# TheProParadox/3dspa_code

Measured on AMD Instinct MI355X. Metric: train-step tracks/sec (B x N_tracks) at T=150, C=772, higher is better.
Workload: dtype bf16

## Files before the change

### 3dspa_code_amd/_lib.py

```python
from __future__ import annotations

import ctypes as C
import os

HERE = os.path.dirname(os.path.abspath(__file__))
LIB_PATH = os.path.join(HERE, 'libspa3d_hip.so')

F32, BF16, F16 = 0, 1, 2


class Config(C.Structure):
  _fields_ = [
      ('num_output_frames', C.c_int32), ('num_latent_tokens', C.c_int32), ('latent_token_dim', C.c_int32),
      ('num_frequencies', C.c_int32), ('track_scale_factor', C.c_float), ('time_scale_factor', C.c_float),
      ('track_token_dim', C.c_int32), ('encoder_latent_dim', C.c_int32), ('decoder_num_channels', C.c_int32),
      ('dino_feature_dim', C.c_int32), ('depth_feature_dim', C.c_int32), ('num_heads', C.c_int32),
      ('qkv_size', C.c_int32), ('enc_mlp', C.c_int32), ('enc_layers', C.c_int32), ('t2l_mlp', C.c_int32),
      ('t2l_layers', C.c_int32), ('dec_mlp', C.c_int32), ('dec_layers', C.c_int32), ('ro_mlp', C.c_int32),
      ('ro_layers', C.c_int32), ('precision', C.c_int32), ('model_kind', C.c_int32),
  ]


class Batch(C.Structure):
  _fields_ = [
# ... 17 lines not shown

class LossConfig(C.Structure):
  _fields_ = [('l1_weight', C.c_float), ('bce_weight', C.c_float), ('position_kind', C.c_int32), ('huber_delta', C.c_float),
              ('axis_weight', C.c_float * 3), ('bce_pos_weight', C.c_float)]


class TapVid3D(C.Structure):
  _fields_ = [('scaling', C.c_int32), ('fixed_thresholds', C.c_int32), ('intrinsics', C.c_void_p), ('query_stats', C.c_void_p),
              ('sample_stats', C.c_void_p), ('scale', C.c_void_p), ('row_scale', C.c_void_p), ('ratio', C.c_void_p)]


class Render(C.Structure):
  _fields_ = [('N', C.c_int32), ('T', C.c_int32), ('H', C.c_int32), ('W', C.c_int32), ('video', C.c_void_p), ('out', C.c_void_p), ('tracks', C.c_void_p),
              ('coords', C.c_int32), ('intrinsics', C.c_void_p), ('extrinsics', C.c_void_p), ('resize_h', C.c_int32), ('resize_w', C.c_int32),
              ('scores', C.c_void_p), ('visible', C.c_void_p), ('normalize', C.c_int32), ('use_visibility', C.c_int32), ('colour_bgr', C.c_int32),
              ('trail', C.c_int32), ('point_size', C.c_int32), ('pixels', C.c_void_p)]


class Clip(C.Structure):
  _fields_ = [('n_tracks', C.c_int32), ('T', C.c_int32), ('H', C.c_int32), ('W', C.c_int32), ('tracks_2d', C.c_void_p), ('tracks_3d', C.c_void_p),
              ('visible', C.c_void_p), ('depth_map', C.c_void_p), ('dino_map', C.c_void_p), ('Hp', C.c_int32), ('Wp', C.c_int32), ('dino_pool', C.c_void_p),
              ('depth_pool', C.c_void_p), ('intrinsics', C.POINTER(C.c_double)), ('n_support', C.c_int32), ('n_query', C.c_int32),
              ('support_index', C.c_void_p), ('query_index', C.c_void_p), ('query_frame', C.c_void_p)]


_SIGS = {
    'spa3d_version': (C.c_char_p, []),
    'spa3d_create': (C.c_int, [C.POINTER(Config), C.POINTER(C.c_void_p)]),
    'spa3d_destroy': (C.c_int, [C.c_void_p]),
    'spa3d_last_error': (C.c_char_p, [C.c_void_p]),
    'spa3d_param_elems': (C.c_int64, [C.c_void_p]),
    'spa3d_num_leaves': (C.c_int32, [C.c_void_p]),
    'spa3d_leaf_info': (C.c_int, [C.c_void_p, C.c_int32, C.c_char_p, C.POINTER(C.c_int32), C.POINTER(C.c_int64),
                                  C.POINTER(C.c_int64)]),
    'spa3d_workspace_bytes': (C.c_int64, [C.c_void_p, C.c_int32, C.c_int32, C.c_int32, C.c_int32, C.c_int32, C.c_int32]),
    'spa3d_encode': (C.c_int, [C.c_void_p, C.c_void_p, C.POINTER(Batch), C.c_void_p, C.c_void_p, C.c_int64, C.c_void_p]),
    'spa3d_decode': (C.c_int, [C.c_void_p, C.c_void_p, C.POINTER(Batch), C.c_void_p, C.POINTER(Outputs), C.c_void_p,
                               C.c_int64, C.c_void_p]),
    'spa3d_forward': (C.c_int, [C.c_void_p, C.c_void_p, C.POINTER(Batch), C.POINTER(Outputs), C.c_void_p, C.c_int64,
                                C.c_void_p]),
    'spa3d_loss': (C.c_int, [C.c_void_p, C.POINTER(Batch), C.POINTER(Outputs), C.c_float, C.c_void_p, C.c_void_p]),
    'spa3d_score': (C.c_int, [C.c_void_p, C.c_void_p, C.POINTER(Batch), C.POINTER(Scores), C.POINTER(Outputs), C.c_void_p, C.c_int64,
                              C.c_void_p]),
    'spa3d_score_folds_workspace_bytes': (C.c_int64, [C.c_void_p, C.c_int32, C.c_int32, C.c_int32]),
    'spa3d_score_folds': (C.c_int, [C.c_void_p, C.c_void_p, C.POINTER(Batch), C.c_int32, C.POINTER(C.c_int32), C.POINTER(Scores), C.POINTER(Outputs),
                                    C.c_void_p, C.c_int64, C.c_void_p]),
    'spa3d_score_from_preds': (C.c_int, [C.c_void_p, C.POINTER(Batch), C.POINTER(Outputs), C.POINTER(Scores), C.c_void_p]),
    'spa3d_tapvid3d_workspace_bytes': (C.c_int64, [C.c_void_p, C.c_int32, C.c_int32, C.c_int32]),
    'spa3d_tapvid3d_from_preds': (C.c_int, [C.c_void_p, C.POINTER(Batch), C.POINTER(Outputs), C.POINTER(TapVid3D), C.c_void_p, C.c_int64, C.c_void_p]),
    'spa3d_render_workspace_bytes': (C.c_int64, [C.c_void_p, C.c_int32, C.c_int32]),
    'spa3d_render_tracks': (C.c_int, [C.c_void_p, C.POINTER(Render), C.c_void_p, C.c_int64, C.c_void_p]),
    'spa3d_build_batch': (C.c_int, [C.c_void_p, C.POINTER(Clip), C.POINTER(Batch), C.c_void_p]),
    'spa3d_op_median_rows': (C.c_int, [C.c_void_p, C.c_int64, C.c_int64, C.c_void_p, C.c_void_p, C.c_int64, C.c_void_p]),
    'spa3d_loss_and_grads': (C.c_int, [C.c_void_p, C.c_void_p, C.POINTER(Batch), C.c_float, C.c_void_p, C.c_int32,
                                       C.c_void_p, C.POINTER(Outputs), C.c_void_p, C.c_int64, C.c_void_p]),
    'spa3d_adamw_step': (C.c_int, [C.c_void_p, C.c_void_p, C.c_void_p, C.c_void_p, C.c_int64, C.c_float, C.c_int64,
                                   C.c_float, C.c_float, C.c_float, C.c_float, C.c_float, C.c_void_p, C.c_void_p]),
    'spa3d_set_option': (C.c_int, [C.c_void_p, C.c_char_p, C.c_double]),
    'spa3d_set_loss_scale_state': (C.c_int, [C.c_void_p, C.c_void_p]),
    'spa3d_set_counts': (C.c_int, [C.c_void_p, C.c_int32, C.POINTER(C.c_int32), C.POINTER(C.c_int32)]),
    'spa3d_set_loss': (C.c_int, [C.c_void_p, C.POINTER(LossConfig)]),
    'spa3d_get_loss': (C.c_int, [C.c_void_p, C.POINTER(LossConfig)]),
    'spa3d_set_point_weights': (C.c_int, [C.c_void_p, C.c_int32, C.c_int32, C.c_void_p]),
    'spa3d_grad_segments': (C.c_int, [C.c_void_p, C.POINTER(C.c_int64)]),
    'spa3d_trainable_range': (C.c_int, [C.c_void_p, C.POINTER(C.c_int64)]),
    'spa3d_set_grad_events': (C.c_int, [C.c_void_p, C.c_void_p, C.c_void_p]),
    'spa3d_grad_events_recorded': (C.c_int, [C.c_void_p, C.POINTER(C.c_int64)]),
    'spa3d_detach': (C.c_int, [C.c_void_p, C.c_void_p, C.c_void_p, C.c_void_p]),
    'spa3d_plan_stats': (C.c_int, [C.c_void_p, C.POINTER(C.c_double)]),
    'spa3d_prof_enable': (C.c_int, [C.c_void_p, C.c_int32]),
    'spa3d_prof_read': (C.c_int, [C.c_void_p, C.c_int32, C.POINTER(C.c_double)]),
    'spa3d_prof_dump': (C.c_int, [C.c_void_p, C.c_char_p]),
    'spa3d_uniform_noise': (C.c_int, [C.c_void_p, C.c_int64, C.c_uint32, C.c_uint32, C.c_void_p]),
    'spa3d_op_sin_embed': (C.c_int, [C.c_void_p, C.c_int64, C.c_int32, C.c_int32, C.c_void_p, C.c_int32, C.c_void_p]),
    'spa3d_op_linear': (C.c_int, [C.c_void_p, C.c_void_p, C.c_void_p, C.c_void_p, C.c_void_p, C.c_int64, C.c_int32,
                                  C.c_int32, C.c_int32, C.c_int32, C.c_int32, C.c_void_p, C.c_int64, C.c_void_p]),
    'spa3d_op_linear_bwd': (C.c_int, [C.c_void_p, C.c_void_p, C.c_void_p, C.c_void_p, C.c_void_p, C.c_void_p, C.c_int64,
                                      C.c_int32, C.c_int32, C.c_int32, C.c_int32, C.c_void_p, C.c_int64, C.c_void_p]),
    'spa3d_op_mlp_fused': (C.c_int, [C.c_void_p] * 9 + [C.c_int64, C.c_int32, C.c_int32, C.c_int32, C.c_void_p, C.c_int64, C.c_void_p]),
    'spa3d_op_layernorm': (C.c_int, [C.c_void_p, C.c_void_p, C.c_void_p, C.c_void_p, C.c_int64, C.c_int32, C.c_int32,
                                     C.c_void_p]),
    'spa3d_op_layernorm_bwd': (C.c_int, [C.c_void_p, C.c_void_p, C.c_void_p, C.c_void_p, C.c_void_p, C.c_void_p,
                                         C.c_int64, C.c_int32, C.c_int32, C.c_void_p]),
    'spa3d_op_qkv_attention': (C.c_int, [C.c_void_p, C.c_int64] + [C.c_void_p] * 7 + [C.c_int64, C.c_int32, C.c_int32] + [C.c_void_p] * 3
                               + [C.c_int32, C.c_void_p, C.c_int64, C.c_void_p]),
    'spa3d_op_attention': (C.c_int, [C.c_void_p] * 3 + [C.c_int64] * 3 + [C.c_void_p] * 3 + [C.c_int64] + [C.c_int32] * 4
                           + [C.c_void_p, C.c_void_p, C.c_int32, C.c_int32, C.c_void_p, C.c_int64, C.c_void_p]),
    'spa3d_op_attention_holdout': (C.c_int, [C.c_void_p] * 3 + [C.c_int64] * 3 + [C.c_void_p] * 2 + [C.c_int64] + [C.c_int32] * 4
                                   + [C.POINTER(C.c_int32), C.c_void_p, C.c_void_p, C.c_int32, C.c_int32, C.c_void_p, C.c_int64, C.c_void_p]),
    'spa3d_op_attention_bwd': (C.c_int, [C.c_void_p] * 3 + [C.c_int64] * 3 + [C.c_void_p] * 3 + [C.c_int64]
                               + [C.c_int32] * 4 + [C.c_void_p] * 8 + [C.c_int32, C.c_int32, C.c_void_p, C.c_int64,
                                                                       C.c_void_p]),
    'spa3d_op_attention_ragged': (C.c_int, [C.c_void_p] * 3 + [C.c_int64] * 3 + [C.c_void_p] * 3 + [C.POINTER(C.c_int32), C.c_int64] + [C.c_int32] * 3
                                  + [C.c_void_p, C.c_void_p, C.c_int32, C.c_int32, C.c_void_p, C.c_int64, C.c_void_p]),
    'spa3d_op_attention_ragged_bwd': (C.c_int, [C.c_void_p] * 3 + [C.c_int64] * 3 + [C.c_void_p] * 3 + [C.POINTER(C.c_int32), C.c_int64] + [C.c_int32] * 3
                                      + [C.c_void_p] * 8 + [C.c_int32, C.c_int32, C.c_void_p, C.c_int64, C.c_void_p]),
    'spa3d_op_attention_varlen': (C.c_int, [C.c_void_p] * 3 + [C.c_int64] * 3 + [C.c_void_p] * 2 + [C.POINTER(C.c_int32), C.c_int64] + [C.c_int32] * 3
                                  + [C.c_void_p, C.c_void_p, C.c_int32, C.c_int32, C.c_void_p, C.c_int64, C.c_void_p]),
    'spa3d_op_attention_varlen_bwd': (C.c_int, [C.c_void_p] * 3 + [C.c_int64] * 3 + [C.c_void_p] * 2 + [C.POINTER(C.c_int32), C.c_int64] + [C.c_int32] * 3
                                      + [C.c_void_p] * 8 + [C.c_int32, C.c_int32, C.c_void_p, C.c_int64, C.c_void_p]),
    'spa3d_op_attention_q1': (C.c_int, [C.c_void_p, C.c_int64, C.c_void_p, C.c_void_p, C.c_int64, C.c_int64] + [C.c_void_p] * 4 + [C.c_int64]
                              + [C.c_int32] * 3 + [C.c_void_p, C.c_void_p, C.c_int32, C.c_void_p]),
    'spa3d_op_attention_q1_bwd': (C.c_int, [C.c_void_p, C.c_int64, C.c_void_p, C.c_void_p, C.c_int64, C.c_int64] + [C.c_void_p] * 4 + [C.c_int64]
                                  + [C.c_int32] * 3 + [C.c_void_p] * 7 + [C.c_int32, C.c_void_p]),
    'spa3d_op_rank_linear': (C.c_int, [C.c_void_p] * 4 + [C.c_int64, C.c_int32, C.c_int32, C.c_int64, C.c_int32, C.c_int32, C.c_int32, C.c_void_p]),
    'spa3d_op_rank_linear_bwd': (C.c_int, [C.c_void_p, C.c_void_p, C.c_int64, C.c_int32, C.c_int32, C.c_int64, C.c_int32, C.c_int32, C.c_void_p,
                                           C.c_void_p, C.c_int32, C.c_void_p]),
    'spa3d_op_colsum': (C.c_int, [C.c_void_p, C.c_int64, C.c_int32, C.c_int64, C.c_int32, C.c_int32, C.c_void_p, C.c_int32, C.c_void_p]),
    'spa3d_op_rows': (C.c_int, [C.c_int32, C.c_void_p, C.c_void_p, C.c_int64, C.c_void_p, C.c_int64, C.c_int32, C.c_int32, C.c_void_p]),
    'spa3d_op_prune_plan': (C.c_int, [C.c_void_p, C.c_int64, C.c_int32, C.c_void_p, C.c_void_p, C.c_void_p, C.POINTER(C.c_int64), C.c_void_p]),
    'spa3d_op_share_plan': (C.c_int, [C.c_void_p, C.c_int64, C.c_int32] + [C.c_void_p] * 5 + [C.POINTER(C.c_int64), C.c_void_p]),
    'spa3d_op_share_rows': (C.c_int, [C.c_int32] + [C.c_void_p] * 6 + [C.c_int64, C.c_int64] + [C.c_int32] * 4 + [C.c_void_p, C.c_int32, C.c_void_p]),
    'spa3d_op_assemble_readout': (C.c_int, [C.c_void_p] * 3 + [C.c_int64] + [C.c_int32] * 4 + [C.c_void_p, C.c_int32, C.c_void_p]),
    'spa3d_op_assemble_readout_bwd': (C.c_int, [C.c_void_p] * 2 + [C.c_int64] + [C.c_int32] * 4 + [C.c_void_p, C.c_void_p, C.c_int32, C.c_int32, C.c_void_p]),
    'spa3d_op_broadcast_rows': (C.c_int, [C.c_void_p, C.c_int32, C.c_int32, C.c_void_p, C.c_int64, C.c_int32, C.c_void_p]),
    'spa3d_op_bcast_grad': (C.c_int, [C.c_void_p, C.c_int64, C.c_int64, C.c_int64, C.c_void_p, C.c_int32, C.c_void_p]),
    'spa3d_op_vis_mean_pool': (C.c_int, [C.c_void_p, C.c_void_p, C.c_int64, C.c_int32, C.c_int32, C.c_void_p, C.c_int32, C.c_void_p]),
    'spa3d_op_vis_mean_pool_bwd': (C.c_int, [C.c_void_p, C.c_void_p, C.c_int64, C.c_int32, C.c_int32, C.c_void_p, C.c_int32, C.c_void_p]),
    'spa3d_op_sin_embed_scaled': (C.c_int, [C.c_void_p, C.c_int64, C.c_int32, C.c_int32, C.c_float, C.c_void_p, C.c_int32, C.c_void_p]),
    'spa3d_op_embed_tokens': (C.c_int, [C.c_void_p, C.c_int64, C.c_int32, C.c_int32, C.c_int32, C.c_float, C.c_void_p, C.c_int32, C.c_void_p]),
    'spa3d_op_query_embed': (C.c_int, [C.c_void_p, C.c_int64, C.c_int32, C.c_int32, C.c_float, C.c_float, C.c_void_p, C.c_void_p, C.c_void_p]),
    'spa3d_op_embed_maps': (C.c_int, [C.c_void_p, C.c_int64, C.c_int32, C.c_int32] + [C.c_void_p] * 4 + [C.c_int32, C.c_int32, C.c_void_p]),
    'spa3d_op_set_readout_rows': (C.c_int, [C.c_void_p, C.c_void_p, C.c_int64, C.c_int32, C.c_int32, C.c_int32, C.c_void_p]),
    'spa3d_op_keymask': (C.c_int, [C.c_void_p, C.c_void_p, C.c_int64, C.c_int32, C.c_int32, C.c_int32, C.c_void_p, C.c_void_p]),
    'spa3d_op_sum3': (C.c_int, [C.c_void_p] * 4 + [C.c_int32, C.c_void_p]),
    'spa3d_op_pack': (C.c_int, [C.c_void_p, C.c_int64, C.c_int32, C.c_int32, C.c_void_p, C.c_int64, C.c_void_p, C.c_int64, C.c_int32, C.c_void_p]),
    'spa3d_op_transpose': (C.c_int, [C.c_void_p, C.c_int32, C.c_int32, C.c_void_p, C.c_int32, C.c_void_p]),
    'spa3d_op_discretize': (C.c_int, [C.c_void_p, C.c_void_p, C.c_int32, C.c_void_p, C.c_void_p, C.c_int64, C.c_void_p]),
    'spa3d_op_sample_dino': (C.c_int, [C.c_void_p, C.c_void_p] + [C.c_int32] * 7 + [C.c_void_p, C.c_int32, C.c_void_p]),
    'spa3d_op_sample_depth_features': (C.c_int, [C.c_void_p, C.c_void_p] + [C.c_int32] * 4 + [C.c_void_p, C.c_void_p]),
    'spa3d_op_lift_2d_to_3d': (C.c_int, [C.c_void_p, C.c_void_p] + [C.c_int32] * 4 + [C.POINTER(C.c_double), C.c_void_p, C.c_void_p]),
}

_lib = None


def exported_symbols():
  return sorted(_SIGS)


def load():
  global _lib
  if _lib is not None:
    return _lib
  if not os.path.exists(LIB_PATH):
    raise ImportError(
        f'{LIB_PATH} is missing: build it with `python -c "import __graft_entry__ as g; g.build()"` '
        '(hipcc --offload-arch=gfx950).  The 3DSPA hot path has no CPU fallback.')
  lib = C.CDLL(LIB_PATH)
  for name, (res, args) in _SIGS.items():
    fn = getattr(lib, name)
    fn.restype = res
    fn.argtypes = args
  _lib = lib
  return lib


class Spa3dError(RuntimeError):
  pass


def check(rc, handle=None, what=''):
  if rc != 0:
    msg = ''
    if handle is not None:
      msg = load().spa3d_last_error(handle).decode()
# ... 2 lines not shown
```

### 3dspa_code_amd/csrc/common.hpp

```cpp
#pragma once
#include <hip/hip_runtime.h>
#include <stdint.h>
#include <algorithm>
#include <string>
#include <vector>

#include "../../include/spa3d.h"
#include "ablate.inc"
#include "gemm_plan.hpp"
#include "attn_plan.hpp"
#include "score_row.hpp"
#include "loss_point.hpp"

#ifndef SPA_F16
#define SPA_F16 0
#endif
#if SPA_F16
#define SPA_NS h_f16
#else
#define SPA_NS h_bf16
#endif
typedef unsigned short bf16_t;

struct DetCfg { float* gbase; long long* shadow; long long n; unsigned* flag; float scale; };
// ... 118 lines not shown

struct ScoreArgs {
  const float* head; const float* tracks; const float* vlog;
  const float* tgt; const float* tvis; const float* scale;
  float* qstats; float* frame_err;
  int64_t nq, row0; int Q, T, NC; ScoreThr thr;
};

constexpr int RENDER_CHUNK = 256;

struct Leaf {
  std::string name;
  int ndim;
  int64_t shape[4];
  int64_t offset;
  int64_t numel() const { int64_t n = 1; for (int i = 0; i < ndim; ++i) n *= shape[i]; return n; }
};

struct Arena {
  char* base = nullptr;
  int64_t cap = 0, off = 0, peak = 0;
  bool dry = false, overflow = false;
  void* alloc(int64_t bytes) {
    int64_t a = (off + 255) & ~int64_t(255);
    off = a + bytes;
    if (off > peak) peak = off;
    if (dry) return (void*)(uintptr_t)(0x1000 + a);
    if (off > cap) { overflow = true; return base; }
    return base + a;
  }
  int64_t mark() const { return off; }
  void release(int64_t m) { off = m; }
};

enum { PROF_GEMM_NT = 0, PROF_GEMM_TN = 1, PROF_GEMM_GENERIC = 2, PROF_ATTN_FWD = 3, PROF_ATTN_BWD = 4, PROF_LN_FWD = 5, PROF_LN_BWD = 6,
       PROF_ATTN_Q1 = 7, PROF_EMBED = 8, PROF_NCLS = 9 };
struct ProfRec { int cls; double flops, bytes; hipEvent_t e0, e1; int64_t tag[4] = {0, 0, 0, 0}; };
struct Prof {
  bool on = false;
  std::vector<hipEvent_t> pool; size_t used = 0;
  std::vector<ProfRec> recs;
  hipEvent_t get() {
    if (used == pool.size()) { hipEvent_t e; if (hipEventCreate(&e) != hipSuccess) return nullptr; pool.push_back(e); }
    return pool[used++];
  }
};

inline spa3d_loss_config loss_config_defaults() {
  spa3d_loss_config d;
  d.l1_weight = 5000.0f; d.bce_weight = 1e-8f; d.position_kind = SPA3D_POS_L1; d.huber_delta = 1.f;
  d.axis_weight[0] = d.axis_weight[1] = d.axis_weight[2] = 1.f; d.bce_pos_weight = 1.f;
  return d;
}

struct spa3d_ctx {
  spa3d_config cfg;
  std::vector<Leaf> leaves;
  int64_t nparams = 0;
  std::string err;
  hipStream_t stream = nullptr;
  Arena ar;
  bool dry = false;
  int hip_err = 0;
  GemmPolicy gemm;
  AttnPolicy attn;
  int chunk = 0;
  int query_chunk = 0;
  int track_chunk = 0;
  int ro_share = 1;
  int prune = 1;
  float loss_scale = 1.f;
  void* grad_ev[2] = {nullptr, nullptr};
  int64_t grad_ev_gen[2] = {0, 0};
  bool last_chunk = false;
  const float* loss_scale_state = nullptr;
  double plan_stats[4] = {0, 0, 0, 0};
  int det_grads = 0;
  const DetCfg* det = nullptr;
  std::vector<int32_t> cnt_n, cnt_q; bool has_cnt_n = false, has_cnt_q = false; int cnt_B = 0;
  spa3d_loss_config loss = loss_config_defaults(); float loss_gmax = 5000.f; int loss_gshift = 0;
  const float* pt_w = nullptr; int pt_B = 0, pt_Q = 0;
  int poison = 0;
  int freeze = 0;
  Prof prof;
};

template <typename F> inline int64_t arena_peak(spa3d_ctx* c, F&& body) {
  const Arena saved = c->ar; const bool sd = c->dry;
  c->ar = Arena(); c->ar.dry = true; c->dry = true;
  body();
  const int64_t peak = c->ar.peak;
  c->ar = saved; c->dry = sd;
  return peak;
}
template <typename F> inline int sized_call(spa3d_ctx* c, const char* what, int64_t need, void* ws, int64_t ws_bytes, void* stream, F&& body) {
  if (!ws || ws_bytes < need) { c->err = std::string(what) + ": workspace too small: need " + std::to_string(need) + " bytes"; return SPA3D_ERR_ARG; }
  c->stream = (hipStream_t)stream; c->dry = false;
  c->ar = Arena(); c->ar.base = (char*)ws; c->ar.cap = ws_bytes;
  body();
  if (c->ar.overflow) { c->err = "internal: arena overflow"; return SPA3D_ERR_WORKSPACE; }
  return c->hip_err ? SPA3D_ERR_HIP : SPA3D_OK;
}
inline bool counts_fit_batch(spa3d_ctx* c, int B) {
  if (c->cnt_B == B) return true;
  c->err = "counts were set for B = " + std::to_string(c->cnt_B) + ", this batch has B = " + std::to_string(B);
  return false;
}
inline bool weights_fit_batch(spa3d_ctx* c, int B, int Q) {
  if (!c->pt_w || (c->pt_B == B && c->pt_Q == Q)) return true;
  c->err = "point weights were set for B = " + std::to_string(c->pt_B) + ", Q = " + std::to_string(c->pt_Q) + ", this batch has B = " + std::to_string(B) +
           ", Q = " + std::to_string(Q);
  return false;
}
inline const int32_t* checked_query_counts(spa3d_ctx* c, int B, int Q) {
  if (!counts_fit_batch(c, B)) return nullptr;
  for (int i = 0; i < B; ++i)
    if (c->cnt_q[i] < 0 || c->cnt_q[i] > Q) {
      c->err = "query_count[" + std::to_string(i) + "] = " + std::to_string(c->cnt_q[i]) + " is outside [0, Q = " + std::to_string(Q) + "]";
      return nullptr;
    }
  return c->cnt_q.data();
}
template <typename F> inline void for_each_live_span(const int32_t* cq, int64_t B, int64_t Q, F&& f) {
  if (!cq) { f((int64_t)0, B * Q); return; }
  for (int64_t i = 0; i < B; ++i) f(i * Q, (int64_t)cq[i]);
}

struct ProfScope {
  spa3d_ctx* c; ProfRec r; bool on;
  ProfScope(spa3d_ctx* c_, int cls, double flops, double bytes) : c(c_), on(c_->prof.on && !c_->dry) {
    if (!on) return;
    r.cls = cls; r.flops = flops; r.bytes = bytes; r.e0 = c->prof.get(); r.e1 = c->prof.get();
    if (!r.e0 || !r.e1) { on = false; return; }
    (void)hipEventRecord(r.e0, c->stream);
  }
  void tag(int64_t a, int64_t b, int64_t c2, int64_t d) { r.tag[0] = a; r.tag[1] = b; r.tag[2] = c2; r.tag[3] = d; }
  ~ProfScope() { if (on) { (void)hipEventRecord(r.e1, c->stream); c->prof.recs.push_back(r); } }
};

#define SPA_LAUNCH_CHECK(ctx)                                                     \
  do {                                                                            \
    hipError_t e__ = hipGetLastError();                                           \
    if (e__ != hipSuccess && (ctx)->hip_err == 0) {                               \
      (ctx)->hip_err = (int)e__;                                                  \
      (ctx)->err = std::string("HIP launch failed at ") + __FILE__ + ":" +        \
                   std::to_string(__LINE__) + ": " + hipGetErrorString(e__);      \
    }                                                                             \
  } while (0)

#define GRID1D(n, bs) dim3((unsigned)std::min<int64_t>(((n) + (bs)-1) / (bs), 1 << 20))
static inline int64_t cdiv(int64_t a, int64_t b) { return (a + b - 1) / b; }

namespace SPA_NS {
template <typename T> void gemm_generic(spa3d_ctx* c, const GemmDesc& d);
void gemm_nt_bf16(spa3d_ctx* c, const GemmDesc& d, GemmKernel k);
void gemm_tn_bf16(spa3d_ctx* c, const GemmDesc& d, GemmKernel k);
int64_t gemm_ntb_pack_elems(int K, int N);
template <typename S> void gemm_ntb_pack(spa3d_ctx* c, const S* w, int64_t sk, int64_t sn, int K, int N, bf16_t* wpk);
void gemm_ntb(spa3d_ctx* c, const GemmDesc& d);
int64_t gemm_rs_pack_elems(int N);
template <typename S> void gemm_rs_pack(spa3d_ctx* c, const S* w, int64_t sk, int64_t sn, int N, bf16_t* wpk);
void gemm_rs(spa3d_ctx* c, const GemmDesc& d);
int64_t qkv_attn_pack_elems(int H);
template <typename S> void qkv_attn_pack(spa3d_ctx* c, const S* wq, const S* wk, const S* wv , int E, int H, bf16_t* wpk);
void qkv_attn_launch(spa3d_ctx* c, const AttnDesc& d);
void attn_fused_launch(spa3d_ctx* c, const AttnDesc& d, const AttnPlan& pl, float* const part[2]);
template <typename S> void mlp_fused_pack(spa3d_ctx* c, const S* w_in , const S* w_out , bf16_t* wpk);
int64_t mlp_fused_pack_elems();
void mlp_fused_fwd(spa3d_ctx* c, const bf16_t* na, const bf16_t* a, bf16_t* y, bf16_t* h, bf16_t* hpre, int64_t M, const bf16_t* wpk,
                   const float* b_in, const float* b_out);
template <typename T> void gemm_launch(spa3d_ctx* c, const GemmDesc& d, GemmKernel k) {
  if (c->dry) return;
  if constexpr (sizeof(T) == 2) {
    if (k == GemmKernel::Rs) return gemm_rs(c, d);
    if (k == GemmKernel::Ntb) return gemm_ntb(c, d);
    if (gemm_is_tn(k)) return gemm_tn_bf16(c, d, k);
    if (k != GemmKernel::Generic) return gemm_nt_bf16(c, d, k);
  }
  gemm_generic<T>(c, d);
}

template <typename T> void k_layernorm(spa3d_ctx*, const T* x, const float* scale, T* y, float* stats, int64_t rows, int d);
template <typename T> void k_layernorm_bwd(spa3d_ctx*, const T* x, const float* scale, const float* stats, const T* dy, T* dx,
                                           float* dscale, int64_t rows, int d, const T* add);
template <typename T> void attention_fwd(spa3d_ctx* c, const AttnDesc& d);
template <typename T> void attention_bwd(spa3d_ctx* c, const AttnDesc& d);
void attn_launch(spa3d_ctx* c, const AttnDesc& d, const AttnPlan& pl);
template <typename T> void k_sin_embed(spa3d_ctx*, const float* x, int64_t rows, int C, int nf, float prescale, T* out);
template <typename T> void k_embed_tokens(spa3d_ctx*, const float* tracks, int64_t nrows, int T_, int nf, float prescale, T* sinbuf, int NC = 3);
void k_query_embed1(spa3d_ctx*, const float* qp, int64_t nq, int nf, float track_scale, float time_scale, float* feat, int32_t* qframe,
                    int NC = 3);
template <typename T> void k_embed_maps(spa3d_ctx*, const int32_t* row_src, int64_t rows, int S, int T_, int32_t* arow, int32_t* crow, T* tok, const float* readout, int d);
template <typename T> void k_set_readout_rows(spa3d_ctx*, T* tok, const float* readout, int64_t nseq, int S, int d);
void k_keymask(spa3d_ctx*, const float* visible, const int32_t* boundary, int64_t nseq, int N, int T_, float* km);
void k_keymask2d(spa3d_ctx*, const float* visible, const int32_t* boundary, int64_t nseq, int N, int T_, float* km);
void k_sum3(spa3d_ctx*, const float* a, const float* b, const float* c3, float* out, int n);
template <typename T> bool k_rank_fwd(spa3d_ctx*, const T* x, const T* w , const float* bias, T* out , int64_t M, int N, int K, int64_t ldo,
                                      int rgroup, int rskip);
template <typename T> bool k_rank_bwd(spa3d_ctx*, const T* x, const T* dy, int64_t M, int N, int K, int64_t ldy, int rgroup, int rskip, float* gw ,
                                      float* gb );
template <typename T> void k_pack(spa3d_ctx*, const float* src, int64_t src_ld, int rows, int cols, T* dst_native, int64_t ldn, T* dst_T, int64_t ldt);
template <typename T> void k_transpose(spa3d_ctx*, const T* src, int rows, int cols, T* dst);
void k_zero(spa3d_ctx*, void* p, int64_t bytes);
void k_set_i32(spa3d_ctx*, int32_t* dst, const int32_t* host, int64_t n);
void k_mul(spa3d_ctx*, float* a, const float* b, int64_t n);
template <typename T> void k_cast_from_f32(spa3d_ctx*, const float* src, T* dst, int64_t n);
template <typename T> void k_cast_to_f32(spa3d_ctx*, const T* src, float* dst, int64_t n);
template <typename T> void k_colsum(spa3d_ctx*, const T* x, int64_t rows, int n, int64_t ld, float* out , int rgroup = 0,
                                    int rskip = 0);
template <typename T> void k_gather_rows(spa3d_ctx*, const T* src, int64_t src_stride_rows, T* dst, int64_t n, int d);
template <typename T> void k_rows_idx(spa3d_ctx*, int mode , const T* src, const int32_t* idx, T* dst, int64_t n, int d);
template <typename T> void k_add_rows_strided(spa3d_ctx*, T* dst, const T* src, int64_t dst_stride_rows, int64_t n, int d);
int64_t k_prune_plan(spa3d_ctx*, const float* km, int64_t nseq, int S, int32_t* cnt, int32_t* seq_off, int32_t* row_src);
int64_t k_share_plan(spa3d_ctx*, const int32_t* qframe, int64_t B, int Q, int32_t* slot, int32_t* slot_b, int32_t* slot_f, int32_t* slot_q0, int32_t* scratch);
template <typename T> void k_share_assemble(spa3d_ctx*, const T* qtok, const T* lat, const int32_t* slot_b, const int32_t* slot_f, int64_t nslot, int64_t BQ,
                                            int L, int Cl, int D, T* xU);
template <typename T> void k_share_expand(spa3d_ctx*, const T* srcU, const int32_t* slot, const int32_t* slot_q0, int64_t nslot, int64_t nseq, int S, int d,
                                          const T* add, T* dst);
template <typename T> void k_share_reduce(spa3d_ctx*, const T* src, const int32_t* slot, const int32_t* slot_b, int64_t nslot, int64_t nseq, int Q, int S, int d,
                                          T* dstU);
template <typename T> void k_assemble_readout(spa3d_ctx*, const T* qtok, const T* lat, const int32_t* qframe, int64_t B, int Q, int L, int Cl,
                                              int D, T* seq);
template <typename T> void k_assemble_readout_bwd(spa3d_ctx*, const T* dseq, const int32_t* qframe, int64_t B, int Q, int L, int Cl, int D,
                                                  T* dqtok, float* dlat, bool accumulate = false);
template <typename T> void k_broadcast_rows(spa3d_ctx*, const float* src, int rows, int d, T* dst, int64_t B);
template <typename T> void k_bcast_grad(spa3d_ctx*, const T* dsrc, int64_t per, int64_t B, int64_t bstride, float* dparam);
template <typename T> void k_vis_mean_pool(spa3d_ctx*, const T* tok, const float* vis, int64_t nseq, int T_, int d, T* out);
template <typename T> void k_vis_mean_pool_bwd(spa3d_ctx*, const T* dout, const float* vis, int64_t nseq, int T_, int d, T* dtok);
template <typename T> void k_attn_q1_fwd(spa3d_ctx*, const T* q0, int64_t ldq0, const T* k, const T* v, int64_t ldk, int64_t ldv,
                                         const float* sq, const float* sk, const float* km, int64_t nseq, int S, int H, int Dh, T* o0,
                                         float* p0, const int32_t* seq_off = nullptr);
template <typename T> void k_attn_q1_bwd(spa3d_ctx*, const T* q0, int64_t ldq0, const T* k, const T* v, int64_t ldk, int64_t ldv,
                                         const float* sq, const float* sk, const float* km, int64_t nseq, int S, int H, int Dh,
                                         const float* p0, const T* d_o0, T* dq0, T* dk, T* dv, float* dsq, float* dsk,
                                         const int32_t* seq_off = nullptr);
void k_discretize(spa3d_ctx*, const float* lat, const float* noise, int discretize, float* out, float* clipmask, int64_t n);
void k_loss_fwd(spa3d_ctx*, const float* head, int64_t nq, int T_, const float* tgt, const float* tvis, float* tracks, float* vlog,
                float* clog, float* sums, unsigned* poison, int NC, const spa3d_loss_config& lc, const float* wgt);
void k_loss_from_preds(spa3d_ctx*, const float* tracks, const float* vlog, int64_t n, const float* tgt, const float* tvis, float* sums,
                       unsigned* poison, int NC, const spa3d_loss_config& lc, const float* wgt);
void k_score_rows(spa3d_ctx*, const ScoreArgs& a);
void k_score_reduce(spa3d_ctx*, const float* qstats, int64_t B, int Q, int K, double* out );
void k_vis_count(spa3d_ctx*, const float* tvis, int64_t n, float* out, unsigned* poison);
void k_set_denom(spa3d_ctx*, const float* sums, const unsigned* poison, float denom_host, float* denom_dev);
void k_loss_finalize(spa3d_ctx*, const float* sums, const unsigned* poison, const float* denom_dev, float l1w, float bcew, float* loss3);
template <typename T> void k_loss_bwd(spa3d_ctx*, const float* head, int64_t nq, int T_, const float* tgt, const float* tvis,
                                      const float* denom_dev, const spa3d_loss_config& lc, const float* wgt, T* dhead, int NC = 3,
                                      const float* scale_dev = nullptr);
void k_set_loss_scale(spa3d_ctx*, const float* denom_dev, float gmax, float setting, float* scale_dev);
void k_unscale(spa3d_ctx*, float* a, const float* scale_dev, int64_t n);
void k_adamw(spa3d_ctx*, float* p, const float* g, float* m, float* v, int64_t n, float lr, int64_t step, float clip, float b1, float b2,
             float eps, float wd, float* scratch);
void k_uniform_noise(spa3d_ctx*, float* out, int64_t n, uint32_t k0, uint32_t k1);
void k_det_flush(spa3d_ctx* c, int64_t lo, int64_t n);
void k_det_unit(spa3d_ctx*, const float* sums, const unsigned* poison, const float* denom_dev, const float* scale_dev, int gshift, const DetCfg& d, DetCfg* out);
}
using namespace SPA_NS;
```

### 3dspa_code_amd/csrc/layernorm.hip

```cpp
#include <algorithm>

#include "common.hpp"

namespace SPA_NS {

template <typename T>
__global__ __launch_bounds__(256) void ln_fwd_kernel(const T* __restrict__ x, const float* __restrict__ scale, T* __restrict__ y,
                                                     float* __restrict__ stats, int64_t rows, int d) {
  const int lane = threadIdx.x & 63;
  int64_t row = (int64_t)blockIdx.x * 4 + (threadIdx.x >> 6);
  const int64_t stride = (int64_t)gridDim.x * 4;
  for (; row < rows; row += stride) {
    const T* xr = x + row * d;
    float s = 0.f, ss = 0.f;
    for (int i = lane; i < d; i += 64) { float v = ld(xr + i); s += v; ss += v * v; }
    s = wave_sum(s); ss = wave_sum(ss);
    float mu = s / d;
    float var = fmaxf(ss / d - mu * mu, 0.f);
    float r = rsqrtf(var + 1e-6f);
    if (stats && lane == 0) { stats[row * 2] = mu; stats[row * 2 + 1] = r; }
    T* yr = y + row * d;
    for (int i = lane; i < d; i += 64) st(yr + i, (ld(xr + i) - mu) * r * scale[i]);
  }
}
#define LN_MAXJ 32
template <typename T>
__global__ __launch_bounds__(256) void ln_bwd_kernel(const T* __restrict__ x, const float* __restrict__ scale,
                                                     const float* __restrict__ stats, const T* __restrict__ dy, const T* add,
                                                     T* dx, float* __restrict__ dscale, int64_t rows, int d, const DetCfg* det) {
  __shared__ float red[4][64 * LN_MAXJ / 4];
  const int lane = threadIdx.x & 63, w = threadIdx.x >> 6;
  float acc[LN_MAXJ];
#pragma unroll
  for (int j = 0; j < LN_MAXJ; ++j) acc[j] = 0.f;
  int64_t row = (int64_t)blockIdx.x * 4 + w;
  const int64_t stride = (int64_t)gridDim.x * 4;
  for (; row < rows; row += stride) {
    const T* xr = x + row * d;
    const T* dyr = dy + row * d;
    const float mu = stats[row * 2], r = stats[row * 2 + 1];
    float sg = 0.f, sgx = 0.f;
#pragma unroll
    for (int j = 0; j < LN_MAXJ; ++j) {
      int i = lane + 64 * j;
      if (i < d) {
        float xh = (ld(xr + i) - mu) * r;
        float dyv = ld(dyr + i);
        float g = dyv * scale[i];
        sg += g; sgx += g * xh;
        acc[j] += dyv * xh;
      }
    }
    sg = wave_sum(sg) / d; sgx = wave_sum(sgx) / d;
    T* dxr = dx + row * d;
#pragma unroll
    for (int j = 0; j < LN_MAXJ; ++j) {
      int i = lane + 64 * j;
      if (i < d) {
        float xh = (ld(xr + i) - mu) * r;
        float g = ld(dyr + i) * scale[i];
        float v = r * (g - sg - xh * sgx);
        if (add) v += ld(add + row * d + i);
        st(dxr + i, v);
      }
    }
  }
  for (int j0 = 0; j0 < LN_MAXJ; j0 += 8) {
    if (j0 * 64 >= d) break;
    __syncthreads();
#pragma unroll
    for (int j = 0; j < 8; ++j) red[w][j * 64 + lane] = acc[j0 + j];
    __syncthreads();
    if (w == 0) {
#pragma unroll
      for (int j = 0; j < 8; ++j) {
        int i = lane + 64 * (j0 + j);
        if (i < d) {
          float s = red[0][j * 64 + lane] + red[1][j * 64 + lane] + red[2][j * 64 + lane] + red[3][j * 64 + lane];
          grad_add(det_read(det), dscale + i, s);
        }
      }
    }
  }
}
template <typename T, int NV>
__device__ __forceinline__ void unpack_vec(const uint4& v, float (&f)[NV]) {
  if constexpr (sizeof(T) == 4) { f[0] = __uint_as_float(v.x); f[1] = __uint_as_float(v.y); f[2] = __uint_as_float(v.z); f[3] = __uint_as_float(v.w); }
  else { const unsigned u[4] = {v.x, v.y, v.z, v.w};
#pragma unroll
    for (int i = 0; i < 4; ++i) { f[2 * i] = unpack_lo(u[i]); f[2 * i + 1] = unpack_hi(u[i]); } }
}
template <typename T, int STEPS, int U = 2>
__global__ __launch_bounds__(256) void ln_fwd_vec_kernel(const T* __restrict__ x, const float* __restrict__ scale, T* __restrict__ y,
                                                         float* __restrict__ stats, int64_t rows, int d) {
  constexpr int NV = VecOf<T>::N;
  const int lane = threadIdx.x & 63, w = threadIdx.x >> 6;
  const int nch = d / NV;
  float sc[STEPS][NV];
#pragma unroll
  for (int s_ = 0; s_ < STEPS; ++s_) {
    const int c = lane + 64 * s_;
#pragma unroll
    for (int j = 0; j < NV; ++j) sc[s_][j] = c < nch ? scale[c * NV + j] : 0.f;
  }
  const int64_t stride = (int64_t)gridDim.x * 4;
  for (int64_t row0 = (int64_t)blockIdx.x * 4 + w; row0 < rows; row0 += stride * U) {
    float xv[U][STEPS][NV];
#pragma unroll
    for (int u = 0; u < U; ++u) {
      const int64_t row = row0 + u * stride;
#pragma unroll
      for (int s_ = 0; s_ < STEPS; ++s_) {
        const int c = lane + 64 * s_;
        if (row < rows && c < nch) load_vec<T, NV>(x + row * d + c * NV, xv[u][s_]);
        else {
#pragma unroll
          for (int j = 0; j < NV; ++j) xv[u][s_][j] = 0.f;
        }
      }
    }
#pragma unroll
    for (int u = 0; u < U; ++u) {
      const int64_t row = row0 + u * stride;
      float s = 0.f, ss = 0.f;
#pragma unroll
      for (int s_ = 0; s_ < STEPS; ++s_)
#pragma unroll
        for (int j = 0; j < NV; ++j) { s += xv[u][s_][j]; ss += xv[u][s_][j] * xv[u][s_][j]; }
      s = wave_sum(s); ss = wave_sum(ss);
      const float mu = s / d;
      const float var = fmaxf(ss / d - mu * mu, 0.f);
      const float r = rsqrtf(var + 1e-6f);
      if (row < rows) {
        if (stats && lane == 0) { stats[row * 2] = mu; stats[row * 2 + 1] = r; }
#pragma unroll
        for (int s_ = 0; s_ < STEPS; ++s_) {
          const int c = lane + 64 * s_;
          if (c < nch) {
            float o[NV];
#pragma unroll
            for (int j = 0; j < NV; ++j) o[j] = (xv[u][s_][j] - mu) * r * sc[s_][j];
            store_vec<T, NV>(y + row * d + c * NV, o);
          }
        }
      }
    }
  }
}
template <typename T, int LPR, int CH>
__global__ __launch_bounds__(256) void ln_fwd_part_kernel(const T* __restrict__ x, const float* __restrict__ scale, T* __restrict__ y,
                                                          float* __restrict__ stats, int64_t rows, int d) {
  constexpr int NV = VecOf<T>::N, RPB = 256 / LPR;
  const int sub = threadIdx.x & (LPR - 1);
  float sc[CH][NV];
#pragma unroll
  for (int c = 0; c < CH; ++c)
#pragma unroll
    for (int j = 0; j < NV; ++j) sc[c][j] = scale[(sub + LPR * c) * NV + j];
  for (int64_t row = (int64_t)blockIdx.x * RPB + threadIdx.x / LPR; row < rows; row += (int64_t)gridDim.x * RPB) {
    uint4 xr[CH];
#pragma unroll
    for (int c = 0; c < CH; ++c) xr[c] = *(const uint4*)(x + row * d + (sub + LPR * c) * NV);
    float xv[CH][NV]; float s = 0.f, ss = 0.f;
#pragma unroll
    for (int c = 0; c < CH; ++c) {
      unpack_vec<T, NV>(xr[c], xv[c]);
#pragma unroll
      for (int j = 0; j < NV; ++j) { s += xv[c][j]; ss += xv[c][j] * xv[c][j]; }
    }
#pragma unroll
    for (int o = 1; o < LPR; o <<= 1) { s += __shfl_xor(s, o, 64); ss += __shfl_xor(ss, o, 64); }
    const float mu = s / d;
    const float var = fmaxf(ss / d - mu * mu, 0.f);
    const float r = rsqrtf(var + 1e-6f);
    if (stats && sub == 0) { stats[row * 2] = mu; stats[row * 2 + 1] = r; }
#pragma unroll
    for (int c = 0; c < CH; ++c) {
      float o[NV];
#pragma unroll
      for (int j = 0; j < NV; ++j) o[j] = (xv[c][j] - mu) * r * sc[c][j];
      store_vec<T, NV>(y + row * d + (sub + LPR * c) * NV, o);
    }
  }
}
template <typename T, int LPR, int CH>
__global__ __launch_bounds__(256) void ln_bwd_part_kernel(const T* __restrict__ x, const float* __restrict__ scale, const float* __restrict__ stats,
                                                          const T* __restrict__ dy, const T* add, T* dx, float* __restrict__ dscale, int64_t rows, int d,
                                                          const DetCfg* det) {
  constexpr int NV = VecOf<T>::N, RPB = 256 / LPR, DV = LPR * CH * NV;
  __shared__ float red[4][DV];
  const int lane = threadIdx.x & 63, w = threadIdx.x >> 6, sub = threadIdx.x & (LPR - 1);
  float acc[CH][NV], sc[CH][NV];
#pragma unroll
  for (int c = 0; c < CH; ++c)
#pragma unroll
    for (int j = 0; j < NV; ++j) { acc[c][j] = 0.f; sc[c][j] = scale[(sub + LPR * c) * NV + j]; }
  for (int64_t row = (int64_t)blockIdx.x * RPB + threadIdx.x / LPR; row < rows; row += (int64_t)gridDim.x * RPB) {
    uint4 xr[CH], dr[CH], ar[CH];
    const float mu = stats[row * 2], r = stats[row * 2 + 1];
#pragma unroll
    for (int c = 0; c < CH; ++c) {
      const int64_t o = row * d + (sub + LPR * c) * NV;
      xr[c] = *(const uint4*)(x + o); dr[c] = *(const uint4*)(dy + o);
      ar[c] = add ? *(const uint4*)(add + o) : make_uint4(0u, 0u, 0u, 0u);
    }
    float xh[CH][NV], gg[CH][NV]; float sg = 0.f, sgx = 0.f;
#pragma unroll
    for (int c = 0; c < CH; ++c) {
      float xv[NV], dv[NV];
      unpack_vec<T, NV>(xr[c], xv); unpack_vec<T, NV>(dr[c], dv);
#pragma unroll
      for (int j = 0; j < NV; ++j) {
        xh[c][j] = (xv[j] - mu) * r; gg[c][j] = dv[j] * sc[c][j];
        sg += gg[c][j]; sgx += gg[c][j] * xh[c][j]; acc[c][j] += dv[j] * xh[c][j];
      }
    }
#pragma unroll
    for (int o = 1; o < LPR; o <<= 1) { sg += __shfl_xor(sg, o, 64); sgx += __shfl_xor(sgx, o, 64); }
    sg /= d; sgx /= d;
#pragma unroll
    for (int c = 0; c < CH; ++c) {
      float o[NV], av[NV];
      unpack_vec<T, NV>(ar[c], av);
#pragma unroll
      for (int j = 0; j < NV; ++j) o[j] = r * (gg[c][j] - sg - xh[c][j] * sgx) + av[j];
      store_vec<T, NV>(dx + row * d + (sub + LPR * c) * NV, o);
    }
  }
#pragma unroll
  for (int c = 0; c < CH; ++c)
#pragma unroll
    for (int j = 0; j < NV; ++j) {
      float a = acc[c][j];
#pragma unroll
      for (int o = LPR; o < 64; o <<= 1) a += __shfl_xor(a, o, 64);
      if (lane < LPR) red[w][(sub + LPR * c) * NV + j] = a;
    }
  __syncthreads();
  for (int t = threadIdx.x; t < DV; t += 256) grad_add(det_read(det), dscale + t, red[0][t] + red[1][t] + red[2][t] + red[3][t]);
}
template <typename T>
void k_layernorm(spa3d_ctx* c, const T* x, const float* scale, T* y, float* stats, int64_t rows, int d) {
  if (c->dry || rows == 0) return;
  ProfScope ps(c, PROF_LN_FWD, 8.0 * (double)rows * d, (double)rows * d * 2.0 * sizeof(T) + rows * 8.0);
  ps.tag(rows, d, 0, 0);
  constexpr int NV = VecOf<T>::N;
  const bool al = ((((uintptr_t)x) | ((uintptr_t)y)) & 15) == 0;
  if (d % NV == 0 && al && d <= 64 * NV * 4) {
    constexpr int gcap = 4096;
    const unsigned g = (unsigned)std::min<int64_t>(cdiv(rows, 8), gcap);
    const int steps = (d / NV + 63) / 64;
    if constexpr (sizeof(T) == 2) {
      if (d == 384) { ln_fwd_part_kernel<T, 16, 3><<<(unsigned)std::min<int64_t>(cdiv(rows, 16), 2 * gcap), 256, 0, c->stream>>>(x, scale, y, stats, rows, d); SPA_LAUNCH_CHECK(c); return; }
      if (d == 1280) { ln_fwd_part_kernel<T, 32, 5><<<(unsigned)std::min<int64_t>(cdiv(rows, 8), 2 * gcap), 256, 0, c->stream>>>(x, scale, y, stats, rows, d); SPA_LAUNCH_CHECK(c); return; }
    }
    if (steps == 1) ln_fwd_vec_kernel<T, 1><<<g, 256, 0, c->stream>>>(x, scale, y, stats, rows, d);
    else if (steps == 2) ln_fwd_vec_kernel<T, 2><<<g, 256, 0, c->stream>>>(x, scale, y, stats, rows, d);
    else if (steps == 3) ln_fwd_vec_kernel<T, 3><<<g, 256, 0, c->stream>>>(x, scale, y, stats, rows, d);
    else ln_fwd_vec_kernel<T, 4><<<g, 256, 0, c->stream>>>(x, scale, y, stats, rows, d);
  } else {
    const unsigned g = (unsigned)std::min<int64_t>(cdiv(rows, 4), 65536);
    ln_fwd_kernel<T><<<g, 256, 0, c->stream>>>(x, scale, y, stats, rows, d);
  }
  SPA_LAUNCH_CHECK(c);
}

template <typename T, int STEPS, int U>
__global__ __launch_bounds__(256) void ln_bwd_vec_kernel(const T* __restrict__ x, const float* __restrict__ scale,
                                                         const float* __restrict__ stats, const T* __restrict__ dy, const T* add, T* dx,
                                                         float* __restrict__ dscale, int64_t rows, int d, const DetCfg* det) {
  constexpr int NV = VecOf<T>::N;
  __shared__ float red[4][64 * NV];
  const int lane = threadIdx.x & 63, w = threadIdx.x >> 6;
  const int nch = d / NV;
  float acc[STEPS][NV], sc[STEPS][NV];
#pragma unroll
  for (int s_ = 0; s_ < STEPS; ++s_) {
    const int c = lane + 64 * s_;
#pragma unroll
    for (int j = 0; j < NV; ++j) { acc[s_][j] = 0.f; sc[s_][j] = c < nch ? scale[c * NV + j] : 0.f; }
  }
  const int64_t stride = (int64_t)gridDim.x * 4;
  for (int64_t row0 = (int64_t)blockIdx.x * 4 + w; row0 < rows; row0 += stride * U) {
    uint4 xr[U][STEPS], dr[U][STEPS], ar[U][STEPS]; float mu[U], r[U];
#pragma unroll
    for (int u = 0; u < U; ++u) {
      const int64_t row = row0 + u * stride;
      const bool live = row < rows;
      mu[u] = live ? stats[row * 2] : 0.f; r[u] = live ? stats[row * 2 + 1] : 0.f;
#pragma unroll
      for (int s_ = 0; s_ < STEPS; ++s_) {
        const int c = lane + 64 * s_;
        xr[u][s_] = dr[u][s_] = ar[u][s_] = make_uint4(0u, 0u, 0u, 0u);
        if (live && c < nch) {
          xr[u][s_] = *(const uint4*)(x + row * d + c * NV); dr[u][s_] = *(const uint4*)(dy + row * d + c * NV);
          if (add) ar[u][s_] = *(const uint4*)(add + row * d + c * NV);
        }
      }
    }
#pragma unroll
    for (int u = 0; u < U; ++u) {
      const int64_t row = row0 + u * stride;
      float xh[STEPS][NV], gg[STEPS][NV];
      float sg = 0.f, sgx = 0.f;
#pragma unroll
      for (int s_ = 0; s_ < STEPS; ++s_) {
        float xv[NV], dv[NV];
        unpack_vec<T, NV>(xr[u][s_], xv); unpack_vec<T, NV>(dr[u][s_], dv);
#pragma unroll
        for (int j = 0; j < NV; ++j) {
          xh[s_][j] = (xv[j] - mu[u]) * r[u]; gg[s_][j] = dv[j] * sc[s_][j];
          sg += gg[s_][j]; sgx += gg[s_][j] * xh[s_][j]; acc[s_][j] += dv[j] * xh[s_][j];
        }
      }
      sg = wave_sum(sg) / d; sgx = wave_sum(sgx) / d;
      if (row < rows) {
#pragma unroll
        for (int s_ = 0; s_ < STEPS; ++s_) {
          const int c = lane + 64 * s_;
          if (c < nch) {
            float o[NV], av[NV];
            unpack_vec<T, NV>(ar[u][s_], av);
#pragma unroll
            for (int j = 0; j < NV; ++j) o[j] = r[u] * (gg[s_][j] - sg - xh[s_][j] * sgx) + av[j];
            store_vec<T, NV>(dx + row * d + c * NV, o);
          }
        }
      }
    }
  }
#pragma unroll
  for (int s_ = 0; s_ < STEPS; ++s_) {
    __syncthreads();
#pragma unroll
    for (int j = 0; j < NV; ++j) red[w][lane * NV + j] = acc[s_][j];
    __syncthreads();
    if (w == 0) {
      const int c = lane + 64 * s_;
      if (c < nch)
#pragma unroll
        for (int j = 0; j < NV; ++j)
          grad_add(det_read(det), dscale + c * NV + j, red[0][lane * NV + j] + red[1][lane * NV + j] + red[2][lane * NV + j] + red[3][lane * NV + j]);
    }
  }
}
template <typename T>
void k_layernorm_bwd(spa3d_ctx* c, const T* x, const float* scale, const float* stats, const T* dy, T* dx, float* dscale,
                     int64_t rows, int d, const T* add) {
  if (c->dry || rows == 0) return;
  ProfScope ps(c, PROF_LN_BWD, 16.0 * (double)rows * d, (double)rows * d * (add ? 4.0 : 3.0) * sizeof(T) + rows * 8.0);
  ps.tag(rows, d, add ? 1 : 0, 0);
  constexpr int gcapb = 1024;
  unsigned g = (unsigned)std::min<int64_t>(cdiv(rows, 4), d <= 512 ? gcapb : 2 * gcapb);
  if (rows <= 16384) g = (unsigned)std::min<int64_t>(g, std::max<int64_t>(64, cdiv(rows, 32)));
  constexpr int NV = VecOf<T>::N;
  const bool al = ((((uintptr_t)x) | ((uintptr_t)dy) | ((uintptr_t)dx) | ((uintptr_t)add)) & 15) == 0;
  if (d % NV == 0 && al && d <= 64 * NV * 4) {
    const int steps = (d / NV + 63) / 64;
    if constexpr (sizeof(T) == 2) {
      if (d == 384) { ln_bwd_part_kernel<T, 16, 3><<<(unsigned)std::min<int64_t>(cdiv(rows, 16), 2 * gcapb), 256, 0, c->stream>>>(x, scale, stats, dy, add, dx, dscale, rows, d, c->det); SPA_LAUNCH_CHECK(c); return; }
      if (d == 1280) { ln_bwd_part_kernel<T, 32, 5><<<(unsigned)std::min<int64_t>(cdiv(rows, 8), 2 * gcapb), 256, 0, c->stream>>>(x, scale, stats, dy, add, dx, dscale, rows, d, c->det); SPA_LAUNCH_CHECK(c); return; }
    }
    if (steps == 1) ln_bwd_vec_kernel<T, 1, 1><<<g, 256, 0, c->stream>>>(x, scale, stats, dy, add, dx, dscale, rows, d, c->det);
    else if (steps == 2) ln_bwd_vec_kernel<T, 2, 2><<<g, 256, 0, c->stream>>>(x, scale, stats, dy, add, dx, dscale, rows, d, c->det);
    else if (steps == 3) ln_bwd_vec_kernel<T, 3, 2><<<g, 256, 0, c->stream>>>(x, scale, stats, dy, add, dx, dscale, rows, d, c->det);
    else ln_bwd_vec_kernel<T, 4, 1><<<g, 256, 0, c->stream>>>(x, scale, stats, dy, add, dx, dscale, rows, d, c->det);
  } else {
    ln_bwd_kernel<T><<<g, 256, 0, c->stream>>>(x, scale, stats, dy, add, dx, dscale, rows, d, c->det);
  }
  SPA_LAUNCH_CHECK(c);
}

#define INST_LN(T) \
  template void k_layernorm<T>(spa3d_ctx*, const T*, const float*, T*, float*, int64_t, int);                                        \
  template void k_layernorm_bwd<T>(spa3d_ctx*, const T*, const float*, const float*, const T*, T*, float*, int64_t, int, const T*);
INST_LN(float)
INST_LN(bf16_t)
}
```

### 3dspa_code_amd/csrc/model.hip

```cpp
#include <algorithm>
#include <cmath>
#include <cstring>
#include <map>

#include "common.hpp"
#include <cstdio>

enum { MODE_FORWARD = 0, MODE_TRAIN = 1, MODE_ENCODE = 2, MODE_DECODE = 3 };

struct RunArgs {
  int mode; const float* P; const spa3d_batch* b; float denom; float* G; int accumulate; float* loss3; spa3d_outputs* out;
  const float* latents_in; float* latents_out; int chunk;
  const int32_t* cn; const int32_t* cq;
  const spa3d_scores* score;
  const float* w;
  int nfold; const int32_t* fold_off;
};

namespace SPA_NS {
static inline const float* at_rows(const float* w, int64_t off) { return w ? w + off : nullptr; }

template <typename T> struct Lin {
  T* wn = nullptr;
  T* wt = nullptr;
// ... 92 lines not shown
      std::string b = name + "/layer_" + std::to_string(i);
      BlockW<T> w; w.d = d; w.mlp = mlp; w.cross = kv > 0; w.dkv = kv;
      w.norm_q = p(b + "/norm_q/scale"); w.g_norm_q = gr(b + "/norm_q/scale");
      w.norm_attn = p(b + "/norm_attn/scale"); w.g_norm_attn = gr(b + "/norm_attn/scale");
      std::string s = b + "/self_att";
      w.qkv = make_lin({s + "/dense_query/kernel", s + "/dense_key/kernel", s + "/dense_value/kernel"}, "", d, E);
      w.sq = p(s + "/norm_query/scale"); w.g_sq = gr(s + "/norm_query/scale");
      w.sk = p(s + "/norm_key/scale"); w.g_sk = gr(s + "/norm_key/scale");
      w.out = make_lin({s + "/dense_out/kernel"}, s + "/dense_out/bias", E, d);
      if (kv) {
        std::string x2 = b + "/cross_att";
        w.cq = make_lin({x2 + "/dense_query/kernel"}, "", d, E);
        w.ckv = make_lin({x2 + "/dense_key/kernel", x2 + "/dense_value/kernel"}, "", kv, E);
        w.csq = p(x2 + "/norm_query/scale"); w.g_csq = gr(x2 + "/norm_query/scale");
        w.csk = p(x2 + "/norm_key/scale"); w.g_csk = gr(x2 + "/norm_key/scale");
        w.cout = make_lin({x2 + "/dense_out/kernel"}, x2 + "/dense_out/bias", E, d);
      }
      w.mlp_in = make_lin({b + "/MLP_in/kernel"}, b + "/MLP_in/bias", d, mlp);
      w.mlp_out = make_lin({b + "/MLP_out/kernel"}, b + "/MLP_out/bias", mlp, d);
      if constexpr (sizeof(T) == 2) {
        if (plan_mlp_pack(c->gemm, w.cross, d, mlp)) {
          w.mlp_pk = alloc<T>(mlp_fused_pack_elems());
          mlp_fused_pack<float>(c, w.mlp_in.src[0], w.mlp_out.src[0], w.mlp_pk);
        }
        if (plan_qkv_pack(c->attn, c->gemm.generic, w.cross, d, Dh)) {
          w.qkv_pk = alloc<T>(qkv_attn_pack_elems(H));
          qkv_attn_pack<float>(c, w.qkv.src[0], w.qkv.src[1], w.qkv.src[2], E, H, w.qkv_pk);
        }
      }
      x.blocks.push_back(w);
    }
    x.norm_enc = p(name + "/norm_encoder/scale"); x.g_norm_enc = gr(name + "/norm_encoder/scale");
    return x;
  }
  void pack() {
    zero_page = c->ar.alloc(256); k_zero(c, zero_page, 256);
    const int d = g.track_token_dim, dl = g.encoder_latent_dim, dd = g.decoder_num_channels, nf = g.num_frequencies;
    lat0 = p("initializer/state_init"); g_lat0 = gr("initializer/state_init");
    readout = nullptr; g_readout = nullptr;
    if (!twoD) { readout = p("input_readout_token/state_init"); g_readout = gr("input_readout_token/state_init"); }
    tok = make_lin({"track_token_projection/kernel"}, "track_token_projection/bias", (NC + 1) * 2 * nf, d);
    if (g.dino_feature_dim > 0) dino = make_lin({"dino_projection/kernel"}, "dino_projection/bias", g.dino_feature_dim, d);
    if (g.depth_feature_dim > 0) depth = make_lin({"depth_projection/kernel"}, "depth_projection/bias", g.depth_feature_dim, d);
    if constexpr (sizeof(T) == 2) {
      if (plan_embed_pack(c->gemm, twoD, d, tok.K, g.dino_feature_dim, g.depth_feature_dim)) {
        emb_K = tok.K + (g.dino_feature_dim > 0 ? dino.K : 0);
        emb_wt = alloc<T>((int64_t)d * emb_K); emb_bias = alloc<float>(d);
        k_pack<T>(c, tok.src[0], d, tok.K, d, nullptr, 0, emb_wt, emb_K);
        if (g.dino_feature_dim > 0) k_pack<T>(c, dino.src[0], d, dino.K, d, nullptr, 0, emb_wt + tok.K, emb_K);
        k_sum3(c, tok.bias, g.dino_feature_dim > 0 ? dino.bias : nullptr, g.depth_feature_dim > 0 ? depth.bias : nullptr, emb_bias, d);
      }
    }
    enc = make_xf("input_track_transformer", d, g.enc_mlp, g.enc_layers, 0);
    t2l = make_xf("tracks_to_latents", dl, g.t2l_mlp, g.t2l_layers, d);
    comp = make_lin({"compressor/kernel"}, "compressor/bias", dl, g.latent_token_dim);
    decomp = make_lin({"decompressor/kernel"}, "decompressor/bias", g.latent_token_dim, dd - 128);
    dec = make_xf("decompress_attn", dd - 128, g.dec_mlp, g.dec_layers, 0);
    ro = make_xf("track_readout_attn", dd, g.ro_mlp, g.ro_layers, 0);
    qenc = make_lin({"query_encoder/kernel"}, "query_encoder/bias", (NC * 2 * nf + 1) * 2 * nf, dd);
    pred = make_lin({"track_predictor/kernel"}, "track_predictor/bias", dd, 4 * g.num_output_frames);
  }

  GemmKernel plan(const GemmDesc& d) const { return sizeof(T) == 2 ? plan_gemm(d, c->gemm) : GemmKernel::Generic; }
  void gemm(const GemmDesc& d) { gemm_launch<T>(c, d, plan(d)); }
  void lin_fwd(const Lin<T>& l, const T* X, void* Y, int64_t M, int epi = EPI_NONE, const T* residual = nullptr, int out_f32 = 0,
               int accumulate = 0, int64_t ldx = 0, int64_t ldy = 0, int crow_group = 0, int crow_skip = 0, T* pre_out = nullptr) {
    GemmDesc d{};
    d.A = X; d.B = l.wn; d.C = Y; d.M = M; d.N = l.N; d.K = l.K;
    d.sAm = ldx ? ldx : l.K; d.sAk = 1; d.sBk = l.ldn; d.sBn = 1; d.sCm = ldy ? ldy : l.N;
    d.Bt = l.wt; d.ldBt = l.K; d.rs_pk = l.wpk; d.ntb_pk = l.wnb;
    d.crow_group = crow_group; d.crow_skip = crow_skip; d.pre_out = pre_out;
    d.bias = l.bias; d.epi = epi; d.aux = residual; d.out_f32 = out_f32; d.accumulate = accumulate;
    gemm(d);
  }
  void lin_bwd_x(const Lin<T>& l, const T* dY, T* dX, int64_t M, const T* gelu_pre = nullptr, int accumulate = 0, int64_t lddx = 0) {
    GemmDesc d{};
    d.A = dY; d.B = l.wn; d.C = dX; d.M = M; d.N = l.K; d.K = l.N;
    d.sAm = l.N; d.sAk = 1; d.sBk = 1; d.sBn = l.ldn; d.sCm = lddx ? lddx : l.K;
    d.Bt = l.wn; d.ldBt = l.ldn; d.rs_pk = l.wpk_t; d.ntb_pk = l.wnb_t;
    if (gelu_pre) { d.epi = EPI_MUL_GELU_GRAD; d.aux = gelu_pre; }
    d.accumulate = accumulate;
    gemm(d);
  }
  void lin_bwd_w(const Lin<T>& l, const T* X, const T* dY, int64_t M, int64_t ldx = 0, int brow_group = 0, int brow_skip = 0) {
    if constexpr (sizeof(T) == 2) {
      if (l.nseg > 1 && !l.gb && l.gw[0]) {
        GemmDesc d{};
        d.A = X; d.B = dY; d.C = l.gw[0]; d.M = l.K; d.N = l.N; d.K = M;
        d.sAm = 1; d.sAk = ldx ? ldx : l.K; d.sBk = l.N; d.sBn = 1; d.sCm = l.segw;
        d.out_f32 = 1; d.accumulate = 1; d.zero_page = zero_page; d.brow_group = brow_group; d.brow_skip = brow_skip;
        d.seg_n = l.segw; d.C_seg[0] = l.gw[1]; d.C_seg[1] = l.nseg > 2 ? l.gw[2] : nullptr;
        const GemmKernel k = plan_tn(d, c->gemm);
        if (k != GemmKernel::Refuse) { gemm_launch<T>(c, d, k); return; }
      }
    }
    for (int s = 0; s < l.nseg; ++s) {
      GemmDesc d{};
      d.A = X; d.B = dY + (int64_t)s * l.segw; d.C = l.gw[s]; d.M = l.K; d.N = l.segw; d.K = M;
      d.sAm = 1; d.sAk = ldx ? ldx : l.K; d.sBk = l.N; d.sBn = 1; d.sCm = l.segw;
      d.out_f32 = 1; d.accumulate = 1; d.zero_page = zero_page; d.brow_group = brow_group; d.brow_skip = brow_skip;
      d.colsum_out = l.gb ? l.gb + (int64_t)s * l.segw : nullptr;
      const GemmKernel k = plan(d);
      gemm_launch<T>(c, d, k);
      if (l.gb && !gemm_tn_fuses_colsum(k, d)) k_colsum<T>(c, dY + (int64_t)s * l.segw, M, l.segw, l.N, l.gb + (int64_t)s * l.segw, brow_group, brow_skip);
    }
  }

  AttnDesc self_desc(const BlockW<T>& w, const T* qkv, T* o, float* lse, const float* km, int64_t nseq, int S, const Rag& rg, const T* d_o = nullptr,
                     T* dqkv = nullptr) {
    AttnDesc a;
    a.q = qkv; a.k = qkv + E; a.v = qkv + 2 * E; a.ldq = a.ldk = a.ldv = 3 * E; a.sq = w.sq; a.sk = w.sk; a.km = km; a.o = o; a.lse = lse;
    a.nseq = nseq; a.Sq = a.Sk = S; a.H = H; a.Dh = Dh; a.esz = (int)sizeof(T);
    if (rg.off) { a.layout = AttnLayout::RaggedRows; a.seq_off = rg.off; a.total_rows = rg.rows; }
    if (d_o) { a.d_o = d_o; a.dq = dqkv; a.dk = dqkv + E; a.dv = dqkv + 2 * E; a.dsq = w.g_sq; a.dsk = w.g_sk; }
    return a;
  }
  AttnDesc cross_desc(const BlockW<T>& w, const T* cq, const T* ckv, T* co, float* clse, int64_t nseq, int S, int Skv, const int32_t* koff_h,
                      const int32_t* koff_d, const Holes* hl, const T* d_o = nullptr, T* dcq = nullptr, T* dckv = nullptr) {
    AttnDesc a;
    a.q = cq; a.k = ckv; a.v = ckv + E; a.ldq = E; a.ldk = a.ldv = 2 * E; a.sq = w.csq; a.sk = w.csk; a.o = co; a.lse = clse;
    a.nseq = nseq; a.Sq = S; a.Sk = Skv; a.H = H; a.Dh = Dh; a.esz = (int)sizeof(T);
    if (hl) { a.layout = AttnLayout::Hole; a.holes_host = hl->host; a.holes_dev = hl->dev; a.Nk = hl->Nk; }
    else if (koff_h) { a.layout = AttnLayout::RaggedKeys; a.koff_host = koff_h; a.koff_dev = koff_d; }
    if (d_o) { a.d_o = d_o; a.dq = dcq; a.dk = dckv; a.dv = dckv + E; a.dsq = w.g_csq; a.dsk = w.g_csk; }
    return a;
  }

  void block_fwd(const BlockW<T>& w, const T* x, T* y, int64_t nseq, int S, const float* km, const T* kv, int Skv, BlockStash<T>* st,
                 const Rag& rg = Rag(), const Share<T>* sh = nullptr, const int32_t* koff_h = nullptr, const int32_t* koff_d = nullptr,
                 const Holes* hl = nullptr) {
    const int64_t M = rg.off ? rg.rows : nseq * S, Mg = rg.off ? (M + 7) & ~int64_t(7) : M; const int d = w.d;
    int64_t mk = c->ar.mark();
    T *nq, *qkv; float* st1;
    if (sh && sh->probe) sh = nullptr;
    if (sh) {
      const int64_t MU = sh->rows(nseq, S), MUg = (MU + 7) & ~int64_t(7);
      nq = alloc<T>(MUg * d); st1 = alloc<float>(MU * 2);
      k_layernorm<T>(c, sh->xU, w.norm_q, nq, st1, MU, d);
      qkv = alloc<T>(Mg * 3 * E);
      const int64_t mk2 = c->ar.mark();
      T* qkvU = alloc<T>(MUg * 3 * E);
      lin_fwd(w.qkv, nq, qkvU, MUg);
      k_share_expand<T>(c, qkvU, sh->slot, sh->slot_q0, sh->nslot, nseq, S, 3 * E, nullptr, qkv);
      c->ar.release(mk2);
    } else {
      nq = alloc<T>(Mg * d); st1 = alloc<float>(M * 2);
      k_layernorm<T>(c, x, w.norm_q, nq, st1, M, d);
      qkv = alloc<T>(Mg * 3 * E);
    }
    T* o = alloc<T>(Mg * E); float* lse = alloc<float>(M * H * 2);
    AttnDesc sa = self_desc(w, qkv, o, lse, km, nseq, S, rg);
    if (!sh) { sa.x = nq; sa.ldx = d; sa.d = d; sa.qkv_pk = w.qkv_pk; }
    const AttnPlan qa = plan_qkv_attn(sa, c->attn);
    if (qa.kernel == AttnKernel::QkvFwd) attn_launch(c, sa, qa);
    else {
      if (!sh) lin_fwd(w.qkv, nq, qkv, Mg);
      attention_fwd<T>(c, sa);
    }
    T* a = alloc<T>(Mg * d);
    lin_fwd(w.out, o, a, Mg, EPI_NONE, x);
    T *cq = nullptr, *ckv = nullptr, *co = nullptr; float* clse = nullptr;
    if (w.cross) {
      cq = alloc<T>(M * E); lin_fwd(w.cq, nq, cq, M);
      const int64_t nkv = hl ? hl->Nk : (koff_h ? koff_h[nseq] : nseq * Skv);
      ckv = alloc<T>(nkv * 2 * E); lin_fwd(w.ckv, kv, ckv, nkv);
      co = alloc<T>(M * E); clse = alloc<float>(M * H * 2);
      attention_fwd<T>(c, cross_desc(w, cq, ckv, co, clse, nseq, S, Skv, koff_h, koff_d, hl));
      lin_fwd(w.cout, co, a, M, EPI_NONE, a);
    }
    T* na = alloc<T>(Mg * d); float* st2 = alloc<float>(Mg * 2);
    k_layernorm<T>(c, a, w.norm_attn, na, st2, M, d);
    T* hpre = alloc<T>(Mg * w.mlp); T* h = alloc<T>(Mg * w.mlp);
    bool fused = false;
    if constexpr (sizeof(T) == 2) {
      fused = plan_mlp(c->gemm, Mg, d, w.mlp, w.mlp_pk, w.mlp_in.bias, w.mlp_out.bias, na, a, y, h, hpre) == GemmKernel::MlpFused;
      if (fused && !c->dry) mlp_fused_fwd(c, na, a, y, h, hpre, Mg, w.mlp_pk, w.mlp_in.bias, w.mlp_out.bias);
    }
    if (!fused) {
      lin_fwd(w.mlp_in, na, h, Mg, EPI_GELU, nullptr, 0, 0, 0, 0, 0, 0, hpre);
      lin_fwd(w.mlp_out, h, y, Mg, EPI_NONE, a);
    }
    if (st) { st->x = const_cast<T*>(sh ? sh->xU : x); st->nq = nq; st->qkv = qkv; st->o = o; st->a = a; st->na = na; st->hpre = hpre; st->h = h;
              st->st1 = st1; st->st2 = st2; st->cq = cq; st->ckv = ckv; st->co = co; st->lse = lse; st->clse = clse; st->shared = sh != nullptr; }
    else c->ar.release(mk);
  }
  void block_bwd(const BlockW<T>& w, const BlockStash<T>& s, const T* dy, T* dx, int64_t nseq, int S, const float* km, const T* kv,
                 int Skv, T* dkv, const Rag& rg = Rag(), const Share<T>* sh = nullptr, const int32_t* koff_h = nullptr, const int32_t* koff_d = nullptr) {
    const int64_t M = rg.off ? rg.rows : nseq * S, Mg = rg.off ? (M + 7) & ~int64_t(7) : M; const int d = w.d;
    int64_t mk = c->ar.mark();
    lin_bwd_w(w.mlp_out, s.h, dy, M);
    T* dh = alloc<T>(Mg * w.mlp);
    lin_bwd_x(w.mlp_out, dy, dh, Mg, s.hpre);
    lin_bwd_w(w.mlp_in, s.na, dh, M);
    T* dna = alloc<T>(Mg * d);
    lin_bwd_x(w.mlp_in, dh, dna, Mg);
    T* da = alloc<T>(Mg * d);
    k_layernorm_bwd<T>(c, s.a, w.norm_attn, s.st2, dna, da, w.g_norm_attn, M, d, dy);
    T* dnq = dna;
    lin_bwd_w(w.out, s.o, da, M);
    T* d_o = alloc<T>(Mg * E);
    lin_bwd_x(w.out, da, d_o, Mg);
    T* dqkv = alloc<T>(Mg * 3 * E);
    attention_bwd<T>(c, self_desc(w, s.qkv, s.o, s.lse, km, nseq, S, rg, d_o, dqkv));
    if (sh && sh->probe) {
      const int64_t MUg = (sh->rows(nseq, S) + 7) & ~int64_t(7), mk2 = c->ar.mark();
      (void)alloc<T>(MUg * 3 * E); (void)alloc<T>(MUg * d); (void)alloc<T>(MUg * d);
      c->ar.release(mk2);
      sh = nullptr;
    }
    if (sh) {
      const int64_t MU = sh->rows(nseq, S), MUg = (MU + 7) & ~int64_t(7);
      T* dqkvU = alloc<T>(MUg * 3 * E);
      k_share_reduce<T>(c, dqkv, sh->slot, sh->slot_b, sh->nslot, nseq, sh->Q, S, 3 * E, dqkvU);
      lin_bwd_w(w.qkv, s.nq, dqkvU, MU);
      T* dnU = alloc<T>(MUg * d);
      lin_bwd_x(w.qkv, dqkvU, dnU, MUg);
      T* dxU = alloc<T>(MU * d);
      k_layernorm_bwd<T>(c, s.x, w.norm_q, s.st1, dnU, dxU, w.g_norm_q, MU, d, nullptr);
      k_share_expand<T>(c, dxU, sh->slot, sh->slot_q0, sh->nslot, nseq, S, d, da, dx);
      c->ar.release(mk);
      return;
    }
    lin_bwd_w(w.qkv, s.nq, dqkv, M);
    lin_bwd_x(w.qkv, dqkv, dnq, Mg);
    if (w.cross) {
      lin_bwd_w(w.cout, s.co, da, M);
      lin_bwd_x(w.cout, da, d_o, M);
      T* dcq = dqkv;
      const int64_t nkv = koff_h ? koff_h[nseq] : nseq * Skv;
      T* dckv = alloc<T>(nkv * 2 * E);
      attention_bwd<T>(c, cross_desc(w, s.cq, s.ckv, s.co, s.clse, nseq, S, Skv, koff_h, koff_d, nullptr, d_o, dcq, dckv));
      lin_bwd_w(w.cq, s.nq, dcq, M);
      lin_bwd_x(w.cq, dcq, dnq, M, nullptr, 1);
      lin_bwd_w(w.ckv, kv, dckv, nkv);
      lin_bwd_x(w.ckv, dckv, dkv, nkv, nullptr, 1);
    }
    k_layernorm_bwd<T>(c, s.x, w.norm_q, s.st1, dnq, dx, w.g_norm_q, M, d, da);
    c->ar.release(mk);
  }


  struct LastStash { T *x, *nq, *kv, *q0, *o0, *x0, *a0, *na0, *hpre0, *h0, *nq0 = nullptr; float *st1, *st2, *p0; };
  void block_fwd_last(const BlockW<T>& w, const T* x, T* y0, int64_t nseq, int S, const float* km, LastStash* st, const Rag& rg = Rag()) {
    const int64_t M = rg.off ? rg.rows : nseq * S, Mg = rg.off ? (M + 7) & ~int64_t(7) : M; const int d = w.d;
    const int64_t mk = c->ar.mark();
    const Lin<T> wq = sub_lin(w.qkv, 0, 1), wkv = sub_lin(w.qkv, 1, 2);
    T* nq = alloc<T>(Mg * d); float* st1 = alloc<float>(M * 2);
    k_layernorm<T>(c, x, w.norm_q, nq, st1, M, d);
    T* kv = alloc<T>(Mg * 2 * E);
    lin_fwd(wkv, nq, kv, Mg);
    T* q0 = alloc<T>(nseq * E); T* nq0 = nullptr;
    if (rg.off) {
      nq0 = alloc<T>(nseq * d);
      k_rows_idx<T>(c, 0, nq, rg.off, nq0, nseq, d);
      lin_fwd(wq, nq0, q0, nseq);
    } else {
      lin_fwd(wq, nq, q0, nseq, EPI_NONE, nullptr, 0, 0, (int64_t)S * d);
    }
    T* o0 = alloc<T>(nseq * E); float* p0 = alloc<float>(nseq * H * S);
    k_attn_q1_fwd<T>(c, q0, E, kv, kv + E, 2 * E, 2 * E, w.sq, w.sk, km, nseq, S, H, Dh, o0, p0, rg.off);
    T* x0 = alloc<T>(nseq * d);
    if (rg.off) k_rows_idx<T>(c, 0, x, rg.off, x0, nseq, d); else k_gather_rows<T>(c, x, S, x0, nseq, d);
    T* a0 = alloc<T>(nseq * d);
    lin_fwd(w.out, o0, a0, nseq, EPI_NONE, x0);
    T* na0 = alloc<T>(nseq * d); float* st2 = alloc<float>(nseq * 2);
    k_layernorm<T>(c, a0, w.norm_attn, na0, st2, nseq, d);
    T* hpre0 = alloc<T>(nseq * w.mlp); T* h0 = alloc<T>(nseq * w.mlp);
    lin_fwd(w.mlp_in, na0, h0, nseq, EPI_GELU, nullptr, 0, 0, 0, 0, 0, 0, hpre0);
    lin_fwd(w.mlp_out, h0, y0, nseq, EPI_NONE, a0);
    if (st) { st->x = const_cast<T*>(x); st->nq = nq; st->kv = kv; st->q0 = q0; st->o0 = o0; st->x0 = x0; st->a0 = a0; st->na0 = na0;
              st->hpre0 = hpre0; st->h0 = h0; st->st1 = st1; st->st2 = st2; st->p0 = p0; st->nq0 = nq0; }
    else c->ar.release(mk);
  }
  void block_bwd_last(const BlockW<T>& w, const LastStash& s, const T* dy0, T* dx, int64_t nseq, int S, const float* km, const Rag& rg = Rag()) {
    const int64_t M = rg.off ? rg.rows : nseq * S, Mg = rg.off ? (M + 7) & ~int64_t(7) : M; const int d = w.d;
    const int64_t mk = c->ar.mark();
    const Lin<T> wq = sub_lin(w.qkv, 0, 1), wkv = sub_lin(w.qkv, 1, 2);
    lin_bwd_w(w.mlp_out, s.h0, dy0, nseq);
    T* dh = alloc<T>(nseq * w.mlp);
    lin_bwd_x(w.mlp_out, dy0, dh, nseq, s.hpre0);
    lin_bwd_w(w.mlp_in, s.na0, dh, nseq);
    T* dna = alloc<T>(nseq * d);
    lin_bwd_x(w.mlp_in, dh, dna, nseq);
    T* da0 = alloc<T>(nseq * d);
    k_layernorm_bwd<T>(c, s.a0, w.norm_attn, s.st2, dna, da0, w.g_norm_attn, nseq, d, dy0);
    lin_bwd_w(w.out, s.o0, da0, nseq);
    T* d_o0 = alloc<T>(nseq * E);
    lin_bwd_x(w.out, da0, d_o0, nseq);
    T* dq0 = alloc<T>(nseq * E); T* dkv = alloc<T>(Mg * 2 * E);
    k_attn_q1_bwd<T>(c, s.q0, E, s.kv, s.kv + E, 2 * E, 2 * E, w.sq, w.sk, km, nseq, S, H, Dh, s.p0, d_o0, dq0, dkv, dkv + E, w.g_sq, w.g_sk,
                     rg.off);
    lin_bwd_w(wkv, s.nq, dkv, M);
    T* dnq = alloc<T>(Mg * d);
    lin_bwd_x(wkv, dkv, dnq, Mg);
    if (rg.off) {
      lin_bwd_w(wq, s.nq0, dq0, nseq);
      T* dnq0 = alloc<T>(nseq * d);
      lin_bwd_x(wq, dq0, dnq0, nseq);
      k_rows_idx<T>(c, 2, dnq0, rg.off, dnq, nseq, d);
    } else {
      lin_bwd_w(wq, s.nq, dq0, nseq, (int64_t)S * d);
      lin_bwd_x(wq, dq0, dnq, nseq, nullptr, 1, (int64_t)S * d);
    }
    k_layernorm_bwd<T>(c, s.x, w.norm_q, s.st1, dnq, dx, w.g_norm_q, M, d, nullptr);
    if (rg.off) k_rows_idx<T>(c, 2, da0, rg.off, dx, nseq, d);
    else k_add_rows_strided<T>(c, dx, da0, S, nseq, d);
    c->ar.release(mk);
  }

  struct Chunk {
    int64_t Bc, nseq; int N, Q, T_, S;
    bool ragged = false;
    bool packed = false; std::vector<int32_t> noff, qoff; int32_t* koff_dev = nullptr;
    bool folds = false; std::vector<int32_t> holes_h; int32_t* holes_dev = nullptr; int lat_f0 = 0;
    int64_t nq() const { return packed ? (int64_t)qoff.back() : Bc * Qc; }
    template <typename F> void for_each_query_span(int64_t b0, F&& f) const {
      if (!packed || folds) { f((int64_t)0, b0 * Q + q_off, nq(), (int64_t)0); return; }
      for (int64_t s = 0; s < Bc; ++s) f((int64_t)qoff[s], (b0 + s) * Q, (int64_t)(qoff[s + 1] - qoff[s]), s);
    }
    int Nk = 0;
    int64_t n_off = 0, q_off = 0; int Nc = 0, Qc = 0; bool count_plan = true;
    T* sinbuf; const void* dino; const void* depthf; float* km; T* tok0; std::vector<BlockStash<T>> enc_st; T* enc_last; T* r0; float* st_r0;
    T* enc_out; LastStash enc_lst, ro_lst; T* enc_ln_all = nullptr; float* st_all = nullptr; const float* sup_vis = nullptr;
    Rag enc_rg; int32_t* row_src = nullptr;
    T* lat_in; std::vector<BlockStash<T>> t2l_st; T* t2l_last; float* st_t2l; T* t2l_n; float* latents;
    float* clipmask; float* lat_q; T* lat_qT; T* dec_in; std::vector<BlockStash<T>> dec_st; T* dec_last; float* st_dec; T* latd;
    float* feat; int32_t* qframe; T* sin2; T* qtok; T* seq0; Share<T> ro_sh; bool ro_share = false; std::vector<BlockStash<T>> ro_st; T* ro_last; T* q0; float* st_q0; T* q0n;
    float* head;
  };

  void encode_tracks(Chunk& k, const spa3d_batch* b, int64_t b0, bool train, T* enc_dst = nullptr) {
    const int d = g.track_token_dim, nf = g.num_frequencies, T_ = k.T_, S = k.S;
    const int64_t nseq = k.nseq, trk0 = b0 * k.N + k.n_off;
    const float* tracks = b->support_tracks + trk0 * T_ * NC;
    k.sup_vis = b->support_tracks_visible + trk0 * T_;
    const bool want_dino = !twoD && g.dino_feature_dim > 0 && b->dino_features, want_depth = !twoD && g.depth_feature_dim > 0 && b->depth_features;
    const T* dino_in = want_dino ? (const T*)b->dino_features + trk0 * T_ * g.dino_feature_dim : nullptr;
    const T* depth_in = want_depth ? (const T*)b->depth_features + trk0 * T_ * g.depth_feature_dim : nullptr;
    if (k.packed) {
      float* pt = alloc<float>(nseq * T_ * NC); float* pv = alloc<float>(nseq * T_);
      T* pd = want_dino ? alloc<T>(nseq * T_ * g.dino_feature_dim) : nullptr; T* pz = want_depth ? alloc<T>(nseq * T_ * g.depth_feature_dim) : nullptr;
      for (int64_t s = 0; s < k.Bc; ++s) {
        const int64_t src = (b0 + s) * k.N * T_, dst = (int64_t)k.noff[s] * T_, n = (int64_t)(k.noff[s + 1] - k.noff[s]) * T_;
        copy_dd(pt + dst * NC, b->support_tracks + src * NC, n * NC * 4);
        copy_dd(pv + dst, b->support_tracks_visible + src, n * 4);
        if (pd) copy_dd(pd + dst * g.dino_feature_dim, (const T*)b->dino_features + src * g.dino_feature_dim, n * g.dino_feature_dim * (int64_t)sizeof(T));
        if (pz) copy_dd(pz + dst * g.depth_feature_dim, (const T*)b->depth_features + src * g.depth_feature_dim, n * g.depth_feature_dim * (int64_t)sizeof(T));
      }
      tracks = pt; k.sup_vis = pv; dino_in = pd; depth_in = pz;
    }
    ProfScope* eps = nullptr;
    {
      const double rows_in = (double)nseq * T_, kin = (double)(NC + 1) * 2 * nf + (b->dino_features ? g.dino_feature_dim : 0) + (b->depth_features ? g.depth_feature_dim : 0);
      const double by = rows_in * (NC * 4.0 + 4.0 + ((b->dino_features ? g.dino_feature_dim : 0) + (b->depth_features ? g.depth_feature_dim : 0)) * (double)sizeof(T)) + rows_in * d * (double)sizeof(T);
      eps = new ProfScope(c, PROF_EMBED, 2.0 * rows_in * kin * d, by);
    }
    k.sinbuf = alloc<T>(nseq * T_ * (NC + 1) * 2 * nf);
    k_embed_tokens<T>(c, tracks, nseq * T_, T_, nf, g.track_scale_factor, k.sinbuf, NC);
    k.km = alloc<float>(nseq * S);
    if (k.packed) {
      for (int64_t s = 0; s < k.Bc; ++s) {
        const int n = k.noff[s + 1] - k.noff[s];
        k_keymask(c, k.sup_vis + (int64_t)k.noff[s] * T_, b->boundary_frame + b0 + s, n, n, T_, k.km + (int64_t)k.noff[s] * S);
      }
    }
    else if (twoD) k_keymask2d(c, k.sup_vis, b->boundary_frame + b0, nseq, k.Nc, T_, k.km);
    else k_keymask(c, k.sup_vis, b->boundary_frame + b0, nseq, k.Nc, T_, k.km);
    k.enc_rg = Rag(); k.row_src = nullptr;
    const bool can_prune = !twoD && c->prune && attn_takes_ragged_self(c->attn, S, Dh, (int)sizeof(T));
// ... 137 lines not shown
    k.seq0 = alloc<T>(nq * S * dd);
    if (k.packed) {
      for (int64_t s = 0; s < k.Bc; ++s) {
        const int64_t q0 = k.qoff[s]; const int qs = k.qoff[s + 1] - k.qoff[s];
        if (qs > 0) k_assemble_readout<T>(c, k.qtok + q0 * dd, k.latd + (k.lat_f0 + s) * L * Cl, k.qframe + q0, 1, qs, L, Cl, dd, k.seq0 + q0 * S * dd);
      }
    }
    else k_assemble_readout<T>(c, k.qtok, k.latd, k.qframe, k.Bc, k.Qc, L, Cl, dd, k.seq0);
    x = k.seq0;
    const int nro = (int)ro.blocks.size();
    k.ro_st.resize(nro);
    k.ro_sh = Share<T>(); k.ro_share = false;
    const bool share_ok = sizeof(T) == 2 && c->ro_share && nro >= 2 && dd % 8 == 0 && Cl % 8 == 0;
    if (share_ok && (k.packed || k.Qc < 8) && k.ragged && !c->dry) c->plan_stats[3] += (double)nq;
    if (share_ok && !k.packed && k.Qc >= 8) {
      int32_t* slot = alloc<int32_t>(nq); int32_t* slot_b = alloc<int32_t>(nq); int32_t* slot_f = alloc<int32_t>(nq);
      int32_t* slot_q0 = alloc<int32_t>(nq); int32_t* scratch = alloc<int32_t>(nq + k.Bc + 1);
      Share<T>& sh = k.ro_sh;
      sh.slot = slot; sh.slot_b = slot_b; sh.slot_q0 = slot_q0; sh.Q = k.Qc;
      if (c->dry) { sh.nslot = (int64_t)(SHARE_MAX_FRAC * (double)nq); sh.probe = true; k.ro_share = true; }
      else {
        sh.nslot = k_share_plan(c, k.qframe, k.Bc, k.Qc, slot, slot_b, slot_f, slot_q0, scratch);
        c->plan_stats[2] += (double)sh.nslot; c->plan_stats[3] += (double)nq;
        if ((double)sh.nslot <= SHARE_MAX_FRAC * (double)nq) {
          T* xU = alloc<T>(((sh.rows(nq, S) + 7) & ~int64_t(7)) * dd);
          k_share_assemble<T>(c, k.qtok, k.latd, slot_b, slot_f, sh.nslot, nq, L, Cl, dd, xU);
          sh.xU = xU; k.ro_share = true;
        }
      }
    }
    T* pp[2] = {nullptr, nullptr};
    if (!train && nro > 1) { pp[0] = alloc<T>(nq * S * dd); if (nro > 2) pp[1] = alloc<T>(nq * S * dd); }
    for (int i = 0; i + 1 < nro; ++i) {
      T* y = train ? alloc<T>(nq * S * dd) : pp[i & 1];
      block_fwd(ro.blocks[i], x, y, nq, S, nullptr, nullptr, 0, train ? &k.ro_st[i] : nullptr, Rag(), (i == 0 && k.ro_share) ? &k.ro_sh : nullptr);
      x = y;
    }
    k.ro_last = const_cast<T*>(x);
    k.q0 = alloc<T>(nq * dd); k.st_q0 = alloc<float>(nq * 2); k.q0n = alloc<T>(nq * dd);
    block_fwd_last(ro.blocks[nro - 1], x, k.q0, nq, S, nullptr, train ? &k.ro_lst : nullptr);
    k_layernorm<T>(c, k.q0, ro.norm_enc, k.q0n, k.st_q0, nq, dd);
    k.head = alloc<float>(nq * 4 * g.num_output_frames);
    lin_fwd(pred, k.q0n, k.head, nq, EPI_NONE, nullptr, 1);
  }


  int64_t seg_lo[2] = {0, 0}, seg_hi[2] = {0, 0};
  const float* scale_dev = nullptr;
  const float* ptw = nullptr;
  bool seg_unscaled[2] = {false, false};
  bool seg_frozen[2] = {false, false};
  void grad_segment_done(int i) {
    if (c->dry || !c->last_chunk || !c->grad_ev[i]) return;
    if (c->det && seg_hi[i] > seg_lo[i] && !seg_frozen[i]) k_det_flush(c, seg_lo[i], seg_hi[i] - seg_lo[i]);
    if (c->loss_scale != 1.f && !seg_frozen[i]) {
      if (!scale_dev || seg_hi[i] <= seg_lo[i]) return;
      k_unscale(c, G + seg_lo[i], scale_dev, seg_hi[i] - seg_lo[i]);
      seg_unscaled[i] = true;
    }
    if (hipEventRecord((hipEvent_t)c->grad_ev[i], c->stream) != hipSuccess && !c->hip_err) { c->hip_err = -6; c->err = "recording a gradient-segment event failed"; }
    else c->grad_ev_gen[i] += 1;
  }
  void backward_queries(Chunk& k, const spa3d_batch* b, int64_t b0, const float* denom_dev, float* dlatd32, bool accumulate) {
    const int L = g.num_latent_tokens, dd = g.decoder_num_channels, Cl = dd - 128, To = g.num_output_frames;
    const int64_t nq = k.nq();
    {
      const int S = L + 1;
      const int64_t mk = c->ar.mark();
      T* dhead = alloc<T>(nq * 4 * To);
      k.for_each_query_span(b0, [&](int64_t r, int64_t br, int64_t n, int64_t) {
        k_loss_bwd<T>(c, k.head + r * 4 * To, n, To, b->query_tracks + br * To * NC, b->query_tracks_visible + br * To, denom_dev,
                      c->loss, at_rows(ptw, br * To), dhead + r * 4 * To, NC, c->loss_scale != 1.f ? denom_dev + 1 : nullptr);
      });
      lin_bwd_w(pred, k.q0n, dhead, nq);
      T* dq0n = alloc<T>(nq * dd);
      lin_bwd_x(pred, dhead, dq0n, nq);
      T* dq0 = alloc<T>(nq * dd);
      k_layernorm_bwd<T>(c, k.q0, ro.norm_enc, k.st_q0, dq0n, dq0, ro.g_norm_enc, nq, dd, nullptr);
      T* dqtok = alloc<T>(nq * dd);
      T* dseq = alloc<T>(nq * S * dd);
      const int nro = (int)ro.blocks.size();
      block_bwd_last(ro.blocks[nro - 1], k.ro_lst, dq0, dseq, nq, S, nullptr);
      for (int i = nro - 2; i >= 0; --i)
        block_bwd(ro.blocks[i], k.ro_st[i], dseq, dseq, nq, S, nullptr, nullptr, 0, nullptr, Rag(), (i == 0 && k.ro_share) ? &k.ro_sh : nullptr);
      if (k.packed) {
        for (int64_t s = 0; s < k.Bc; ++s) {
          const int64_t q0 = k.qoff[s]; const int qs = k.qoff[s + 1] - k.qoff[s];
          if (qs > 0) k_assemble_readout_bwd<T>(c, dseq + q0 * S * dd, k.qframe + q0, 1, qs, L, Cl, dd, dqtok + q0 * dd, dlatd32 + s * L * Cl, accumulate);
          else if (!accumulate) k_zero(c, dlatd32 + s * L * Cl, (int64_t)L * Cl * 4);
        }
      }
      else k_assemble_readout_bwd<T>(c, dseq, k.qframe, k.Bc, k.Qc, L, Cl, dd, dqtok, dlatd32, accumulate);
      lin_bwd_w(qenc, k.sin2, dqtok, nq);
      c->ar.release(mk);
    }
  }
  T* backward_latents(Chunk& k, const float* dlatd32, bool lat0_trains = true) {
    const int L = g.num_latent_tokens, Ld = g.latent_token_dim, dd = g.decoder_num_channels, Cl = dd - 128;
    const int d = g.track_token_dim, dl = g.encoder_latent_dim;
    const int64_t nl = k.Bc * L;
    T* ddec = alloc<T>(nl * Cl);
    {
      T* dlatd = alloc<T>(nl * Cl);
      k_cast_from_f32<T>(c, dlatd32, dlatd, nl * Cl);
      k_layernorm_bwd<T>(c, k.dec_last, dec.norm_enc, k.st_dec, dlatd, ddec, dec.g_norm_enc, nl, Cl, nullptr);
    }
    for (int i = (int)dec.blocks.size() - 1; i >= 0; --i)
      block_bwd(dec.blocks[i], k.dec_st[i], ddec, ddec, k.Bc, L, nullptr, nullptr, 0, nullptr);
    lin_bwd_w(decomp, k.lat_qT, ddec, nl);
    T* dlq = alloc<T>(nl * Ld);
    lin_bwd_x(decomp, ddec, dlq, nl);
    float* dl32 = alloc<float>(nl * Ld);
    k_cast_to_f32<T>(c, dlq, dl32, nl * Ld);
    k_mul(c, dl32, k.clipmask, nl * Ld);
    k_cast_from_f32<T>(c, dl32, dlq, nl * Ld);
    lin_bwd_w(comp, k.t2l_n, dlq, nl);
    T* dt2ln = alloc<T>(nl * dl);
    lin_bwd_x(comp, dlq, dt2ln, nl);
    T* dt2l = alloc<T>(nl * dl);
    k_layernorm_bwd<T>(c, k.t2l_last, t2l.norm_enc, k.st_t2l, dt2ln, dt2l, t2l.g_norm_enc, nl, dl, nullptr);
    const int64_t nkeys = k.packed ? (int64_t)k.noff.back() : k.Bc * k.Nk;
    T* denc_out = alloc<T>(nkeys * d);
    k_zero(c, denc_out, nkeys * d * (int64_t)sizeof(T));
    for (int i = (int)t2l.blocks.size() - 1; i >= 0; --i)
      block_bwd(t2l.blocks[i], k.t2l_st[i], dt2l, dt2l, k.Bc, L, nullptr, k.enc_out, k.Nk, denc_out, Rag(), nullptr, k.packed ? k.noff.data() : nullptr, k.koff_dev);
    grad_segment_done(1);
    if (lat0_trains) k_bcast_grad<T>(c, dt2l, (int64_t)L * dl, k.Bc, (int64_t)L * dl, g_lat0);
    return denc_out;
  }
  void backward_tracks(Chunk& k, const T* denc_out) {
    const int d = g.track_token_dim, T_ = k.T_;
    const int64_t nseq = k.nseq;
    const int S = k.S;
    const int64_t erows = k.enc_rg.off ? (k.enc_rg.rows + 7) & ~int64_t(7) : nseq * S;
    T* dtok = alloc<T>(erows * d);
    const int nenc = (int)enc.blocks.size();
    if (twoD) {
      T* dln = alloc<T>(nseq * S * d);
      k_vis_mean_pool_bwd<T>(c, denc_out, k.sup_vis, nseq, T_, d, dln);
      k_layernorm_bwd<T>(c, k.enc_last, enc.norm_enc, k.st_all, dln, dtok, enc.g_norm_enc, nseq * S, d, nullptr);
      for (int i = nenc - 1; i >= 0; --i)
        block_bwd(enc.blocks[i], k.enc_st[i], dtok, dtok, nseq, S, k.km, nullptr, 0, nullptr);
      lin_bwd_w(tok, k.sinbuf, dtok, nseq * T_);
    } else {
      T* dr0 = alloc<T>(nseq * d);
      k_layernorm_bwd<T>(c, k.r0, enc.norm_enc, k.st_r0, denc_out, dr0, enc.g_norm_enc, nseq, d, nullptr);
      const Rag& rg = k.enc_rg;
      const float* km = rg.off ? nullptr : k.km;
      block_bwd_last(enc.blocks[nenc - 1], k.enc_lst, dr0, dtok, nseq, S, km, rg);
      for (int i = nenc - 2; i >= 0; --i)
        block_bwd(enc.blocks[i], k.enc_st[i], dtok, dtok, nseq, S, km, nullptr, 0, nullptr, rg);
      const T* dtok_dense = dtok;
      if (rg.off) {
        T* d0 = alloc<T>(nseq * d);
        k_rows_idx<T>(c, 0, dtok, rg.off, d0, nseq, d);
        k_bcast_grad<T>(c, d0, d, nseq, d, g_readout);
        T* dd = alloc<T>(nseq * S * d);
        k_zero(c, dd, nseq * S * d * (int64_t)sizeof(T));
        k_rows_idx<T>(c, 1, dtok, k.row_src, dd, rg.rows, d);
        dtok_dense = dd;
      } else {
        k_bcast_grad<T>(c, dtok, d, nseq, (int64_t)S * d, g_readout);
      }
      lin_bwd_w(tok, k.sinbuf, dtok_dense, nseq * T_, 0, T_, 1);
      if (k.dino) lin_bwd_w(dino, (const T*)k.dino, dtok_dense, nseq * T_, 0, T_, 1);
      bool streamed = false;
      if constexpr (sizeof(T) == 2)
        streamed = k.depthf && depth.nseg == 1 && k_rank_bwd<T>(c, (const T*)k.depthf, dtok_dense, nseq * T_, depth.N, depth.K, d, T_, 1, depth.gw[0], depth.gb);
      if (k.depthf && !streamed)
        lin_bwd_w(depth, (const T*)k.depthf, dtok_dense, nseq * T_, 0, T_, 1);
    }
  }
};

static void poison_from(spa3d_ctx* c, int64_t mark) {
  if (!c->poison || c->dry) return;
  const int64_t o = (mark + 255) & ~int64_t(255);
  if (o < c->ar.cap) (void)hipMemsetAsync(c->ar.base + o, 0xFF, (size_t)(c->ar.cap - o), c->stream);
}

static ScoreArgs score_args(const spa3d_batch* b, const spa3d_scores* sc, int To, int NC) {
  ScoreArgs s{};
  s.tgt = b->query_tracks; s.tvis = b->query_tracks_visible; s.scale = sc->sample_scale; s.qstats = sc->query_stats; s.frame_err = sc->frame_err;
  s.Q = b->Q; s.T = To; s.NC = NC; s.thr.K = sc->num_thresholds;
  for (int i = 0; i < SCORE_MAX_K; ++i) s.thr.t[i] = i < sc->num_thresholds ? sc->thresholds[i] : 0.f;
  return s;
}
static void score_zero_rows(spa3d_ctx* c, const spa3d_scores* sc, int64_t r0, int64_t nr, int To) {
  if (c->dry || nr <= 0) return;
  const int64_t S = score_row_len(sc->num_thresholds);
  (void)hipMemsetAsync(sc->query_stats + r0 * S, 0, (size_t)(nr * S) * 4, c->stream);
  if (sc->frame_err) (void)hipMemsetAsync(sc->frame_err + r0 * To, 0, (size_t)(nr * To) * 4, c->stream);
}
static void zero_padded_rows(spa3d_ctx* c, const RunArgs& a, int NC, int64_t r0, int64_t nr) {
  if (c->dry || nr <= 0) return;
  const int To = c->cfg.num_output_frames;
  if (a.out && a.out->tracks) (void)hipMemsetAsync(a.out->tracks + r0 * To * NC, 0, (size_t)(nr * To * NC) * 4, c->stream);
  if (a.out && a.out->visible_logits) (void)hipMemsetAsync(a.out->visible_logits + r0 * To, 0, (size_t)(nr * To) * 4, c->stream);
  if (a.out && a.out->certain_logits) (void)hipMemsetAsync(a.out->certain_logits + r0 * To, 0, (size_t)(nr * To) * 4, c->stream);
  if (a.score) score_zero_rows(c, a.score, r0, nr, To);
}

template <typename T>
static void emit_outputs(spa3d_ctx* c, const RunArgs& a, Net<T>& net, typename Net<T>::Chunk& k, int64_t b0, float* sums, unsigned* poison) {
  const spa3d_batch* b = a.b; const int To = c->cfg.num_output_frames, NC = net.NC;
  const bool train = a.mode == MODE_TRAIN;
  if (a.score) {
    ScoreArgs s = score_args(b, a.score, To, NC);
    k.for_each_query_span(b0, [&](int64_t r, int64_t br, int64_t n, int64_t) { s.head = k.head + r * 4 * To; s.nq = n; s.row0 = br; k_score_rows(c, s); });
    if (!a.out) return;
  }
  k.for_each_query_span(b0, [&](int64_t r, int64_t br, int64_t n, int64_t) {
    float* tr = a.out && a.out->tracks ? a.out->tracks + br * To * NC : nullptr;
    float* vl = a.out && a.out->visible_logits ? a.out->visible_logits + br * To : nullptr;
    float* cl = a.out && a.out->certain_logits ? a.out->certain_logits + br * To : nullptr;
    k_loss_fwd(c, k.head + r * 4 * To, n, To, train ? b->query_tracks + br * To * NC : nullptr, train ? b->query_tracks_visible + br * To : nullptr,
               tr, vl, cl, sums, poison, NC, c->loss, train ? at_rows(a.w, br * To) : nullptr);
  });
}

template <typename T>
static void run_chunk(spa3d_ctx* c, const RunArgs& a, Net<T>& net, typename Net<T>::Chunk& k, int64_t b0, const float* noise, float* sums,
                      unsigned* poison, const float* denom_dev) {
  const spa3d_batch* b = a.b; const spa3d_config& g = c->cfg;
  const int L = g.num_latent_tokens, Ld = g.latent_token_dim, Cl = g.decoder_num_channels - 128, d = g.track_token_dim;
  const bool train = a.mode == MODE_TRAIN;
  const bool release_each = c->query_chunk > 0 || c->track_chunk > 0 || (k.ragged && !k.packed);
  const int64_t ntrk = k.nseq, Qall = k.Qc;
  const int64_t tc = c->track_chunk > 0 ? std::min<int64_t>(c->track_chunk, ntrk) : ntrk, qc = c->query_chunk > 0 ? std::min<int64_t>(c->query_chunk, Qall) : Qall;
  auto track_slice = [&](int64_t n0) { k.n_off = n0; k.Nc = (int)std::min(tc, ntrk - n0); k.nseq = k.Nc; };
  const int fz = train ? c->freeze : 0;
  const bool stash_enc = train && fz < 1, stash_lat = train && fz < 2;
  if (a.mode != MODE_DECODE) {
    float* lat_keep = fz >= 2 ? net.template alloc<float>(k.Bc * L * Ld) : nullptr;
// ... 281 lines not shown
  return c->hip_err ? SPA3D_ERR_HIP : SPA3D_OK;
}

static void set_gemm_impl(spa3d_ctx* c, int v) { c->gemm = GemmPolicy::from_impl(v == 7 || v == 10 ? 2 : v); }

static int check_batch(spa3d_ctx* c, const spa3d_batch* b, int mode) {
  if (!b || b->B <= 0 || b->Q <= 0) { c->err = "batch: B,Q must be positive"; return SPA3D_ERR_ARG; }
  if (mode != MODE_DECODE && (b->N <= 0 || b->T <= 0 || !b->support_tracks || !b->support_tracks_visible || !b->boundary_frame)) {
    c->err = "batch: support_tracks / support_tracks_visible / boundary_frame required"; return SPA3D_ERR_ARG;
  }
  if (mode != MODE_ENCODE && !b->query_points) { c->err = "batch: query_points required (host builds the default grid)"; return SPA3D_ERR_ARG; }
  if (mode == MODE_TRAIN && (!b->query_tracks || !b->query_tracks_visible)) { c->err = "batch: targets required"; return SPA3D_ERR_ARG; }
  if (c->cfg.decoder_num_channels - 128 <= 0) { c->err = "decoder_num_channels must exceed 128"; return SPA3D_ERR_ARG; }
  return SPA3D_OK;
}

static int run(spa3d_ctx* c, RunArgs a, void* ws, int64_t ws_bytes, void* stream) {
  c->err.clear(); c->hip_err = 0;
  int rc = check_batch(c, a.b, a.mode);
  if (rc) return rc;
  int lo = 1, hi = a.b->B;
  if (a.chunk <= 0) a.chunk = c->chunk;
  if (c->query_chunk > 0 || c->track_chunk > 0) {
    if (a.chunk > 1) { c->err = "\"chunk\" > 1 cannot be combined with \"query_chunk\" / \"track_chunk\" (they imply one sample per chunk)"; return SPA3D_ERR_ARG; }
    a.chunk = 1;
  }
  a.w = nullptr;
  if (a.mode == MODE_TRAIN) {
    if (!weights_fit_batch(c, a.b->B, a.b->Q)) return SPA3D_ERR_ARG;
    a.w = c->pt_w;
  }
  a.cn = nullptr; a.cq = nullptr;
  if (c->has_cnt_n || c->has_cnt_q) {
    const spa3d_batch* b = a.b;
    if (!counts_fit_batch(c, b->B)) return SPA3D_ERR_ARG;
    if (c->cfg.model_kind == 1) { c->err = "per-sample counts are not supported by the 2-D model (model_kind 1)"; return SPA3D_ERR_ARG; }
    if (c->query_chunk > 0 || c->track_chunk > 0) { c->err = "per-sample counts cannot be combined with \"query_chunk\" / \"track_chunk\""; return SPA3D_ERR_ARG; }
    if (c->has_cnt_n && a.mode != MODE_DECODE) {
      for (int i = 0; i < b->B; ++i)
        if (c->cnt_n[i] < 1 || c->cnt_n[i] > b->N) { c->err = "support_count[" + std::to_string(i) + "] = " + std::to_string(c->cnt_n[i]) + " is outside [1, N = " + std::to_string(b->N) + "]"; return SPA3D_ERR_ARG; }
      a.cn = c->cnt_n.data();
    }
    if (c->has_cnt_q && a.mode != MODE_ENCODE && !(a.cq = checked_query_counts(c, b->B, b->Q))) return SPA3D_ERR_ARG;
    bool full = true;
    for (int i = 0; i < b->B && full; ++i) full = (!a.cn || a.cn[i] == b->N) && (!a.cq || a.cq[i] == b->Q);
    if (full) { a.cn = nullptr; a.cq = nullptr; }
  }
  if (a.chunk > 0) { lo = hi = std::min(a.chunk, a.b->B); }
  return sized_run(c, a, lo, hi, 0, ws, ws_bytes, stream, [&](int64_t need) {
    c->err = "workspace too small: need " + std::to_string(need) + " bytes for chunk " + std::to_string(lo);
    return SPA3D_ERR_WORKSPACE;
  });
}

extern "C" {

const char* spa3d_version(void) { return "spa3d-hip 0.1 (gfx950)"; }

int spa3d_create(const spa3d_config* cfg, spa3d_handle* out) {
  if (!cfg || !out) return SPA3D_ERR_ARG;
  if (cfg->num_heads <= 0 || cfg->qkv_size % cfg->num_heads) return SPA3D_ERR_ARG;
  if (cfg->qkv_size / cfg->num_heads > 128 || cfg->num_frequencies > 64 || cfg->num_frequencies <= 0) return SPA3D_ERR_ARG;
  { const int Dh = cfg->qkv_size / cfg->num_heads;
    if (Dh != 8 && Dh != 16 && Dh != 32 && Dh != 64 && Dh != 96 && Dh != 128) return SPA3D_ERR_ARG; }
  if (cfg->precision != SPA3D_F32 && cfg->precision != SPA3D_BF16 && cfg->precision != SPA3D_F16) return SPA3D_ERR_ARG;
  if (cfg->model_kind != 0 && cfg->model_kind != 1) return SPA3D_ERR_ARG;
  if (cfg->model_kind == 1 && (cfg->dino_feature_dim != 0 || cfg->depth_feature_dim != 0)) return SPA3D_ERR_ARG;
  if (cfg->track_token_dim > 2048 || cfg->decoder_num_channels > 2048 || cfg->encoder_latent_dim > 2048) return SPA3D_ERR_ARG;
  spa3d_ctx* c = new (std::nothrow) spa3d_ctx();
  if (!c) return SPA3D_ERR_ARG;
  c->cfg = *cfg;
  build_leaves(c);
  if (cfg->precision == SPA3D_F16) c->loss_scale = -16.f;
  const char* e = getenv("SPA3D_GEMM_IMPL"); if (e) set_gemm_impl(c, atoi(e));
  e = getenv("SPA3D_ATTN_IMPL"); if (e) c->attn = AttnPolicy::from_impl(atoi(e));
  e = getenv("SPA3D_LOSS_SCALE"); if (e && cfg->precision == SPA3D_F16) c->loss_scale = (float)atof(e);
  e = getenv("SPA3D_PRUNE"); if (e) c->prune = atoi(e);
  e = getenv("SPA3D_RO_SHARE"); if (e) c->ro_share = atoi(e);
  e = getenv("SPA3D_CHUNK"); if (e) c->chunk = atoi(e);
  e = getenv("SPA3D_DET_GRADS"); if (e) c->det_grads = atoi(e) != 0;
  e = getenv("SPA3D_QUERY_CHUNK"); if (e) c->query_chunk = std::max(0, atoi(e));
  e = getenv("SPA3D_TRACK_CHUNK"); if (e) c->track_chunk = std::max(0, atoi(e));
  e = getenv("SPA3D_FREEZE"); if (e && atoi(e) >= 0 && atoi(e) <= 2) c->freeze = atoi(e);
  *out = c;
  return SPA3D_OK;
}
int spa3d_destroy(spa3d_handle h) { delete h; return SPA3D_OK; }
const char* spa3d_last_error(spa3d_handle h) { return h ? h->err.c_str() : "null handle"; }
int64_t spa3d_param_elems(spa3d_handle h) { return h ? h->nparams : 0; }
int32_t spa3d_num_leaves(spa3d_handle h) { return h ? (int32_t)h->leaves.size() : 0; }
int spa3d_leaf_info(spa3d_handle h, int32_t i, char* name, int32_t* ndim, int64_t* shape, int64_t* offset) {
  if (!h || i < 0 || i >= (int32_t)h->leaves.size()) return SPA3D_ERR_ARG;
  const Leaf& l = h->leaves[i];
  if (name) { strncpy(name, l.name.c_str(), 159); name[159] = 0; }
  if (ndim) *ndim = l.ndim;
  if (shape) for (int k = 0; k < l.ndim; ++k) shape[k] = l.shape[k];
  if (offset) *offset = l.offset;
  return SPA3D_OK;
}

int64_t spa3d_workspace_bytes(spa3d_handle h, int32_t B, int32_t N, int32_t Q, int32_t T, int32_t chunk, int32_t train) {
  if (!h || B <= 0 || N <= 0 || Q <= 0 || T <= 0) return -1;
  const spa3d_batch b = sizing_batch(h, B, N, Q, T);
  RunArgs a{}; a.mode = train ? MODE_TRAIN : MODE_FORWARD; a.b = &b; a.G = train ? (float*)0x100000 : nullptr;
  if (h->query_chunk > 0 || h->track_chunk > 0) chunk = 1;
  return dry_need(h, a, std::max(1, std::min(chunk, B)));
}

int spa3d_encode(spa3d_handle h, const float* params, const spa3d_batch* b, float* latents, void* ws, int64_t ws_bytes, void* stream) {
  if (!h || !params || !latents) return SPA3D_ERR_ARG;
  RunArgs a{}; a.mode = MODE_ENCODE; a.P = params; a.b = b; a.latents_out = latents;
  return run(h, a, ws, ws_bytes, stream);
}
int spa3d_decode(spa3d_handle h, const float* params, const spa3d_batch* b, const float* latents, spa3d_outputs* out, void* ws,
                 int64_t ws_bytes, void* stream) {
  if (!h || !params || !latents || !out) return SPA3D_ERR_ARG;
  RunArgs a{}; a.mode = MODE_DECODE; a.P = params; a.b = b; a.latents_in = latents; a.out = out;
  return run(h, a, ws, ws_bytes, stream);
}
int spa3d_forward(spa3d_handle h, const float* params, const spa3d_batch* b, spa3d_outputs* out, void* ws, int64_t ws_bytes, void* stream) {
  if (!h || !params || !out) return SPA3D_ERR_ARG;
  RunArgs a{}; a.mode = MODE_FORWARD; a.P = params; a.b = b; a.out = out;
  return run(h, a, ws, ws_bytes, stream);
}
static int check_scores(spa3d_ctx* c, const spa3d_batch* b, const spa3d_scores* sc) {
  c->err.clear();
  if (!b || !b->query_tracks || !b->query_tracks_visible) { c->err = "score: the batch needs its targets (query_tracks, query_tracks_visible)"; return SPA3D_ERR_ARG; }
  if (!sc || !sc->query_stats) { c->err = "score: spa3d_scores::query_stats is required"; return SPA3D_ERR_ARG; }
  if (sc->num_thresholds < 0 || sc->num_thresholds > SCORE_MAX_K) { c->err = "score: num_thresholds = " + std::to_string(sc->num_thresholds) + " is outside [0, 8]"; return SPA3D_ERR_ARG; }
  for (int i = 0; i < sc->num_thresholds; ++i)
    if (!(std::isfinite(sc->thresholds[i]) && sc->thresholds[i] > 0.f)) { c->err = "score: thresholds[" + std::to_string(i) + "] must be finite and positive"; return SPA3D_ERR_ARG; }
  return SPA3D_OK;
}
int spa3d_score(spa3d_handle h, const float* params, const spa3d_batch* b, spa3d_scores* scores, spa3d_outputs* out, void* ws, int64_t ws_bytes, void* stream) {
  if (!h || !params) return SPA3D_ERR_ARG;
  const int rc = check_scores(h, b, scores);
  if (rc) return rc;
  RunArgs a{}; a.mode = MODE_FORWARD; a.P = params; a.b = b; a.out = out; a.score = scores;
  return run(h, a, ws, ws_bytes, stream);
}
static std::vector<int32_t> equal_folds(int N, int F) {
  std::vector<int32_t> off(1, 0);
  for (int f = 0; f < F; ++f) off.push_back(off.back() + N / F + (f < N % F ? 1 : 0));
  return off;
}
int64_t spa3d_score_folds_workspace_bytes(spa3d_handle h, int32_t N, int32_t T, int32_t num_folds) {
  if (!h || h->cfg.model_kind != 0 || T <= 0 || num_folds < 2 || num_folds > 64 || N < num_folds) return -1;
  const std::vector<int32_t> off = equal_folds(N, num_folds);
  const spa3d_batch b = sizing_batch(h, 1, N, N, T);
  RunArgs a{}; a.mode = MODE_FORWARD; a.b = &b; a.nfold = num_folds; a.fold_off = off.data();
  return dry_need(h, a, 1);
}
int spa3d_score_folds(spa3d_handle h, const float* params, const spa3d_batch* b, int32_t num_folds, const int32_t* fold_off, spa3d_scores* scores,
                      spa3d_outputs* out, void* ws, int64_t ws_bytes, void* stream) {
  if (!h || !params) return SPA3D_ERR_ARG;
  h->err.clear(); h->hip_err = 0;
  auto refuse = [&](const std::string& m) { h->err = "score_folds: " + m; return SPA3D_ERR_ARG; };
  int rc = check_batch(h, b, MODE_FORWARD);
  if (rc) return rc;
  if (b->Q != b->N) return refuse("the batch must have Q == N (query row q of a clip is its track q), got Q = " + std::to_string(b->Q) + ", N = " + std::to_string(b->N));
  if (num_folds < 2 || num_folds > 64) return refuse("num_folds = " + std::to_string(num_folds) + " is outside [2, 64]");
  if (!fold_off) return refuse("fold_off is required");
  if (fold_off[0] != 0 || fold_off[num_folds] != b->N) return refuse("fold_off must start at 0 and end at N = " + std::to_string(b->N));
  for (int f = 0; f < num_folds; ++f)
    if (fold_off[f + 1] <= fold_off[f]) return refuse("fold_off must be strictly increasing (fold_off[" + std::to_string(f + 1) + "] = " + std::to_string(fold_off[f + 1]) + ")");
  spa3d_batch bb = *b;
  if (!bb.query_tracks && !bb.query_tracks_visible) {
    if (b->T != h->cfg.num_output_frames) return refuse("targets left NULL need T == num_output_frames, got T = " + std::to_string(b->T) + ", num_output_frames = " + std::to_string(h->cfg.num_output_frames));
    bb.query_tracks = b->support_tracks; bb.query_tracks_visible = b->support_tracks_visible;
  }
  if (h->cfg.model_kind != 0) return refuse("not supported by the 2-D model (model_kind 1)");
  if (h->has_cnt_n || h->has_cnt_q) return refuse("per-sample counts (spa3d_set_counts) cannot be combined with folds");
  if (h->track_chunk > 0 || h->query_chunk > 0) return refuse("\"track_chunk\" / \"query_chunk\" cannot be combined with folds");
  rc = check_scores(h, &bb, scores);
  if (rc) return rc;
  RunArgs a{}; a.mode = MODE_FORWARD; a.P = params; a.b = &bb; a.out = out; a.score = scores; a.nfold = num_folds; a.fold_off = fold_off;
  return sized_run(h, a, 1, num_folds, spa3d_score_folds_workspace_bytes(h, b->N, b->T, num_folds), ws, ws ? ws_bytes : 0, stream,
                   [&](int64_t need) { return refuse("workspace too small: need " + std::to_string(need) + " bytes"); });
}
int spa3d_score_from_preds(spa3d_handle h, const spa3d_batch* b, const spa3d_outputs* preds, spa3d_scores* scores, void* stream) {
  if (!h) return SPA3D_ERR_ARG;
  h->hip_err = 0;
  const int rc = check_scores(h, b, scores);
  if (rc) return rc;
  if (!preds || !preds->tracks || !preds->visible_logits) { h->err = "score: predictions (tracks, visible_logits) are required"; return SPA3D_ERR_ARG; }
  if (b->B <= 0 || b->Q <= 0) { h->err = "batch: B,Q must be positive"; return SPA3D_ERR_ARG; }
  const int32_t* cq = nullptr;
  if (h->has_cnt_q && !(cq = checked_query_counts(h, b->B, b->Q))) return SPA3D_ERR_ARG;
  h->stream = (hipStream_t)stream; h->dry = false;
  const int To = h->cfg.num_output_frames;
  ScoreArgs s = score_args(b, scores, To, h->cfg.model_kind == 1 ? 2 : 3);
  s.tracks = preds->tracks; s.vlog = preds->visible_logits;
  for_each_live_span(cq, b->B, b->Q, [&](int64_t row0, int64_t nq) {
    s.nq = nq; s.row0 = row0;
    k_score_rows(h, s);
    if (cq) score_zero_rows(h, scores, row0 + nq, b->Q - nq, To);
  });
  if (scores->sample_stats) k_score_reduce(h, scores->query_stats, b->B, b->Q, scores->num_thresholds, scores->sample_stats);
  return h->hip_err ? SPA3D_ERR_HIP : SPA3D_OK;
}

int spa3d_loss_and_grads(spa3d_handle h, const float* params, const spa3d_batch* b, float denom, float* grads, int32_t accumulate,
                         float* loss3, spa3d_outputs* out, void* ws, int64_t ws_bytes, void* stream) {
  if (!h || !params || !grads) return SPA3D_ERR_ARG;
  if (accumulate && h->loss_scale != 1.f) { h->err = "accumulate=1 is not supported with a loss scale (fp16 mode)"; return SPA3D_ERR_ARG; }
  RunArgs a{}; a.mode = MODE_TRAIN; a.P = params; a.b = b; a.denom = denom; a.G = grads; a.accumulate = accumulate; a.loss3 = loss3; a.out = out;
  return run(h, a, ws, ws_bytes, stream);
}

int spa3d_loss(spa3d_handle h, const spa3d_batch* b, const spa3d_outputs* preds, float denom, float* loss3, void* stream) {
  if (!h || !b || !preds || !loss3 || !preds->tracks || !preds->visible_logits || !b->query_tracks || !b->query_tracks_visible)
    return SPA3D_ERR_ARG;
  h->err.clear(); h->hip_err = 0; h->stream = (hipStream_t)stream; h->dry = false;
  if (((uintptr_t)loss3) & 7) { h->err = "loss3 must be 8-byte aligned"; return SPA3D_ERR_ARG; }
  float* scratch = loss3 + 4;
  unsigned* poison = (unsigned*)(loss3 + 3);
  const int To = h->cfg.num_output_frames, NC = h->cfg.model_kind == 1 ? 2 : 3;
  const int32_t* cq = nullptr;
  if (h->has_cnt_q && !(cq = checked_query_counts(h, b->B, b->Q))) return SPA3D_ERR_ARG;
  if (!weights_fit_batch(h, b->B, b->Q)) return SPA3D_ERR_ARG;
  k_zero(h, loss3 + 3, 36);
  for_each_live_span(cq, b->B, b->Q, [&](int64_t row0, int64_t nq) { k_vis_count(h, b->query_tracks_visible + row0 * To, nq * To, scratch + 4, poison); });
  k_set_denom(h, scratch, poison, denom, scratch + 6);
  for_each_live_span(cq, b->B, b->Q, [&](int64_t row0, int64_t nq) {
    const int64_t r = row0 * To;
    k_loss_from_preds(h, preds->tracks + r * NC, preds->visible_logits + r, nq * To, b->query_tracks + r * NC, b->query_tracks_visible + r, scratch, poison, NC,
                      h->loss, at_rows(h->pt_w, r));
  });
  k_loss_finalize(h, scratch, poison, scratch + 6, h->loss.l1_weight, h->loss.bce_weight, loss3);
  return h->hip_err ? SPA3D_ERR_HIP : SPA3D_OK;
}

int spa3d_set_option(spa3d_handle h, const char* name, double value) {
  if (!h || !name) return SPA3D_ERR_ARG;
  const std::string n(name);
  if (n == "prune") h->prune = value != 0;
  else if (n == "ro_share") h->ro_share = value != 0;
  else if (n == "loss_scale") { if (h->cfg.precision != SPA3D_F16) { h->err = "loss_scale applies to SPA3D_F16 handles only"; return SPA3D_ERR_ARG; } h->loss_scale = (float)value; }
  else if (n == "attn_impl") h->attn = AttnPolicy::from_impl((int)value);
  else if (n == "gemm_impl") set_gemm_impl(h, (int)value);
  else if (n == "chunk") {
    if (value > 1 && (h->query_chunk > 0 || h->track_chunk > 0)) { h->err = "\"chunk\" > 1 cannot be combined with \"query_chunk\" / \"track_chunk\""; return SPA3D_ERR_ARG; }
    h->chunk = value > 0 ? (int)value : 0;
  }
  else if (n == "query_chunk" || n == "track_chunk") {
    if (!(value >= 0 && value <= 2147483647.0)) { h->err = n + " must be >= 0"; return SPA3D_ERR_ARG; }
    if (value >= 1 && h->chunk > 1) { h->err = "\"" + n + "\" cannot be combined with \"chunk\" > 1 (it implies one sample per chunk)"; return SPA3D_ERR_ARG; }
    (n == "query_chunk" ? h->query_chunk : h->track_chunk) = (int)value;
  }
  else if (n == "poison") h->poison = value != 0;
  else if (n == "det_grads") h->det_grads = value != 0;
  else if (n == "freeze") {
    if (value != 0 && value != 1 && value != 2) { h->err = "freeze must be 0 (nothing frozen), 1 (track encoder side) or 2 (the latent stacks too)"; return SPA3D_ERR_ARG; }
    h->freeze = (int)value;
  }
  else { h->err = "unknown option: " + n; return SPA3D_ERR_ARG; }
  return SPA3D_OK;
}
int spa3d_set_loss_scale_state(spa3d_handle h, const float* state) {
  if (!h) return SPA3D_ERR_ARG;
  h->loss_scale_state = state;
  return SPA3D_OK;
}
int spa3d_set_counts(spa3d_handle h, int32_t B, const int32_t* support_count, const int32_t* query_count) {
  if (!h) return SPA3D_ERR_ARG;
  h->has_cnt_n = h->has_cnt_q = false; h->cnt_n.clear(); h->cnt_q.clear(); h->cnt_B = 0;
  if (!support_count && !query_count) return SPA3D_OK;
  if (B <= 0) { h->err = "spa3d_set_counts: B must be positive"; return SPA3D_ERR_ARG; }
  h->cnt_B = B;
  if (support_count) { h->cnt_n.assign(support_count, support_count + B); h->has_cnt_n = true; }
  if (query_count) { h->cnt_q.assign(query_count, query_count + B); h->has_cnt_q = true; }
  return SPA3D_OK;
}
int spa3d_set_loss(spa3d_handle h, const spa3d_loss_config* cfg) {
  if (!h) return SPA3D_ERR_ARG;
  const spa3d_loss_config d = cfg ? *cfg : loss_config_defaults();
  const int NC = h->cfg.model_kind == 1 ? 2 : 3;
  auto refuse = [&](const std::string& m) { h->err = "spa3d_set_loss: " + m; return SPA3D_ERR_ARG; };
  if (d.position_kind != SPA3D_POS_L1 && d.position_kind != SPA3D_POS_HUBER) return refuse("position_kind = " + std::to_string(d.position_kind) + " is neither SPA3D_POS_L1 nor SPA3D_POS_HUBER");
  const bool huber = d.position_kind == SPA3D_POS_HUBER;
  bool finite = std::isfinite(d.l1_weight) && std::isfinite(d.bce_weight) && std::isfinite(d.bce_pos_weight) && (!huber || std::isfinite(d.huber_delta));
  for (int i = 0; i < NC; ++i) finite = finite && std::isfinite(d.axis_weight[i]);
  if (!finite) return refuse("every field must be finite");
  bool negative = d.l1_weight < 0.f || d.bce_weight < 0.f || d.bce_pos_weight < 0.f;
  float amax = 0.f;
  for (int i = 0; i < NC; ++i) { negative = negative || d.axis_weight[i] < 0.f; amax = std::max(amax, d.axis_weight[i]); }
  if (negative) return refuse("l1_weight, bce_weight, axis_weight and bce_pos_weight must not be negative");
  if (huber && !(d.huber_delta > 0.f)) return refuse("huber_delta must be positive with SPA3D_POS_HUBER");
  if (d.l1_weight > 0.f && !(amax > 0.f)) return refuse("l1_weight > 0 needs a positive axis_weight among the model's " + std::to_string(NC) + " coordinates");
  const float gmax = std::max(d.l1_weight * amax, d.bce_weight * std::max(1.f, d.bce_pos_weight));
  if (!(gmax > 0.f && gmax <= 1073741824.f)) return refuse("the largest head gradient max(l1_weight * max axis_weight, bce_weight * max(1, bce_pos_weight)) must lie in (0, 2^30]");
  int e = 0;
  (void)frexp((double)gmax / 5000.0, &e);
  h->loss = d; h->loss_gmax = gmax; h->loss_gshift = e - 1;
  return SPA3D_OK;
}
int spa3d_get_loss(spa3d_handle h, spa3d_loss_config* out) {
  if (!h || !out) return SPA3D_ERR_ARG;
  *out = h->loss;
  return SPA3D_OK;
}
int spa3d_set_point_weights(spa3d_handle h, int32_t B, int32_t Q, const float* w) {
  if (!h) return SPA3D_ERR_ARG;
  h->pt_w = nullptr; h->pt_B = h->pt_Q = 0;
  if (!w) return SPA3D_OK;
  if (B <= 0 || Q <= 0) { h->err = "spa3d_set_point_weights: B and Q must be positive"; return SPA3D_ERR_ARG; }
  h->pt_w = w; h->pt_B = B; h->pt_Q = Q;
  return SPA3D_OK;
}
int spa3d_grad_segments(spa3d_handle h, int64_t* bounds4) {
  if (!h || !bounds4) return SPA3D_ERR_ARG;
  int64_t b1 = -1, b2 = -1;
  for (auto& l : h->leaves) {
    if (b1 < 0 && l.name.rfind("tracks_to_latents/", 0) == 0) b1 = l.offset;
    if (b2 < 0 && l.name.rfind("track_readout_attn/", 0) == 0) b2 = l.offset;
  }
  if (b1 < 0 || b2 < b1) return SPA3D_ERR_ARG;
  bounds4[0] = 0; bounds4[1] = b1; bounds4[2] = b2; bounds4[3] = h->nparams;
  return SPA3D_OK;
}
// ... 77 lines not shown
```

### 3dspa_code_amd/csrc/ops.hip

```cpp
#include <cmath>

#include "common.hpp"

namespace SPA_NS {
namespace {
struct OpCtx : spa3d_ctx {
  OpCtx(void* stream_, void* ws, int64_t ws_bytes) {
    stream = (hipStream_t)stream_; ar.base = (char*)ws; ar.cap = ws_bytes;
  }
  template <typename U> U* alloc(int64_t n) { return (U*)ar.alloc(n * (int64_t)sizeof(U)); }
  int status() { return ar.overflow ? SPA3D_ERR_WORKSPACE : (hip_err ? SPA3D_ERR_HIP : SPA3D_OK); }
};

template <typename T>
int op_linear(OpCtx& c, const T* A, const T* B, const float* bias, const T* res, T* C, int64_t M, int N, int K, int act, int impl) {
  GemmDesc d{};
  d.A = A; d.B = B; d.C = C; d.M = M; d.N = N; d.K = K; d.sAm = K; d.sAk = 1; d.sBk = N; d.sBn = 1; d.sCm = N;
  d.bias = bias; d.epi = act == 1 ? EPI_GELU : (act == 2 ? EPI_MUL_GELU_GRAD : EPI_NONE); d.aux = res;
  const GemmPolicy p = GemmPolicy::from_impl(impl & 15);
  if constexpr (sizeof(T) == 2) {
    if (p.only != GemmKernel::Refuse) {
      const bool rs = p.only == GemmKernel::Rs;
      const void*& pk = rs ? d.rs_pk : d.ntb_pk;
      pk = A;
// ... 96 lines not shown
#define OP_BY_DTYPE(dtype, body)                                            \
  do {                                                                      \
    if ((dtype) == SPA3D_F32) { using T = float; body; }                    \
    else { using T = bf16_t; body; }                                        \
  } while (0)
static bool op_al16(const void* p) { return (((uintptr_t)p) & 15) == 0; }
static int op_nv(int32_t dtype) { return dtype == SPA3D_F32 ? 4 : 8; }

extern "C" {

SPA3D_OP(spa3d_op_sin_embed)(const float* x, int64_t rows, int32_t C, int32_t nf, void* out, int32_t dtype, void* stream) {
  FWD16(spa3d_op_sin_embed, x, rows, C, nf, out, dtype, stream)
  if (!x || !out || nf <= 0 || nf > 64) return SPA3D_ERR_ARG;
  OpCtx c(stream, nullptr, 0);
  OP_BY_DTYPE(dtype, k_sin_embed<T>(&c, x, rows, C, nf, 1.0f, (T*)out));
  return c.status();
}

SPA3D_OP(spa3d_op_linear)(const void* A, const void* B, const float* bias, const void* residual, void* C, int64_t M, int32_t N, int32_t K,
                          int32_t act, int32_t dtype, int32_t impl, void* ws, int64_t ws_bytes, void* stream) {
  FWD16(spa3d_op_linear, A, B, bias, residual, C, M, N, K, act, dtype, impl, ws, ws_bytes, stream)
  if (!A || !B || !C) return SPA3D_ERR_ARG;
  OpCtx c(stream, ws, ws_bytes);
  OP_BY_DTYPE(dtype, return op_linear<T>(c, (const T*)A, (const T*)B, bias, (const T*)residual, (T*)C, M, N, K, act, impl));
}
SPA3D_OP(spa3d_op_linear_bwd)(const void* A, const void* B, const void* dC, void* dA, float* dB, float* dbias, int64_t M, int32_t N, int32_t K,
                              int32_t dtype, int32_t impl, void* ws, int64_t ws_bytes, void* stream) {
  FWD16(spa3d_op_linear_bwd, A, B, dC, dA, dB, dbias, M, N, K, dtype, impl, ws, ws_bytes, stream)
  if (!A || !B || !dC) return SPA3D_ERR_ARG;
  OpCtx c(stream, ws, ws_bytes);
  OP_BY_DTYPE(dtype, return op_linear_bwd<T>(c, (const T*)A, (const T*)B, (const T*)dC, (T*)dA, dB, dbias, M, N, K, impl));
}

SPA3D_OP(spa3d_op_mlp_fused)(const void* na, const void* a, const void* w_in, const float* b_in, const void* w_out, const float* b_out, void* y,
                             void* h, void* hpre, int64_t M, int32_t d, int32_t mlp, int32_t dtype, void* ws, int64_t ws_bytes, void* stream) {
  FWD16(spa3d_op_mlp_fused, na, a, w_in, b_in, w_out, b_out, y, h, hpre, M, d, mlp, dtype, ws, ws_bytes, stream)
  if (!na || !a || !w_in || !b_in || !w_out || !b_out || !y || !h || !hpre || dtype == SPA3D_F32) return SPA3D_ERR_ARG;
  if (d != 384 || mlp != 1536 || M < 1) return SPA3D_ERR_ARG;
  for (const void* p : {na, a, (const void*)y, (const void*)h, (const void*)hpre, w_in, w_out})
    if (!op_al16(p)) return SPA3D_ERR_ARG;
  OpCtx c(stream, ws, ws_bytes);
  bf16_t* wpk = c.alloc<bf16_t>(mlp_fused_pack_elems());
  if (c.ar.overflow) return SPA3D_ERR_WORKSPACE;
  mlp_fused_pack<bf16_t>(&c, (const bf16_t*)w_in, (const bf16_t*)w_out, wpk);
  if (plan_mlp(GemmPolicy(), M, d, mlp, wpk, b_in, b_out, na, a, y, h, hpre) != GemmKernel::MlpFused) return SPA3D_ERR_ARG;
  mlp_fused_fwd(&c, (const bf16_t*)na, (const bf16_t*)a, (bf16_t*)y, (bf16_t*)h, (bf16_t*)hpre, M, wpk, b_in, b_out);
  return c.status();
}

SPA3D_OP(spa3d_op_qkv_attention)(const void* nq, int64_t ldn, const void* wq, const void* wk, const void* wv, const float* scale_q, const float* scale_k,
                                 const float* keymask, const int32_t* seq_off, int64_t nseq, int32_t S, int32_t H, void* qkv, void* o, float* lse,
                                 int32_t dtype, void* ws, int64_t ws_bytes, void* stream) {
  FWD16(spa3d_op_qkv_attention, nq, ldn, wq, wk, wv, scale_q, scale_k, keymask, seq_off, nseq, S, H, qkv, o, lse, dtype, ws, ws_bytes, stream)
  if (!nq || !wq || !wk || !wv || !scale_q || !scale_k || !qkv || !o || dtype == SPA3D_F32 || H < 1 || H > 64) return SPA3D_ERR_ARG;
  OpCtx c(stream, ws, ws_bytes);
  bf16_t* wpk = c.alloc<bf16_t>(qkv_attn_pack_elems(H));
  if (c.ar.overflow) return SPA3D_ERR_WORKSPACE;
  qkv_attn_pack<bf16_t>(&c, (const bf16_t*)wq, (const bf16_t*)wk, (const bf16_t*)wv, H * ATTN_DH, H, wpk);
  const int E = H * ATTN_DH;
  AttnDesc a = op_attn_desc(qkv, (const bf16_t*)qkv + E, (const bf16_t*)qkv + 2 * E, 3 * E, 3 * E, 3 * E, scale_q, scale_k, keymask, nseq, S, S, H, ATTN_DH, o, lse, dtype);
  if (seq_off) { a.layout = AttnLayout::RaggedRows; a.seq_off = seq_off; }
  a.x = nq; a.ldx = ldn; a.d = QKVA_D; a.qkv_pk = wpk;
  const AttnPlan pl = plan_qkv_attn(a, AttnPolicy::from_impl(6));
  if (pl.kernel != AttnKernel::QkvFwd) return SPA3D_ERR_ARG;
  attn_launch(&c, a, pl);
  return c.status();
}

SPA3D_OP(spa3d_op_layernorm)(const void* x, const float* scale, void* y, float* stats, int64_t rows, int32_t d, int32_t dtype, void* stream) {
  FWD16(spa3d_op_layernorm, x, scale, y, stats, rows, d, dtype, stream)
  if (!x || !scale || !y || d <= 0 || d > 2048) return SPA3D_ERR_ARG;
  OpCtx c(stream, nullptr, 0);
  OP_BY_DTYPE(dtype, k_layernorm<T>(&c, (const T*)x, scale, (T*)y, stats, rows, d));
  return c.status();
}
SPA3D_OP(spa3d_op_layernorm_bwd)(const void* x, const float* scale, const float* stats, const void* dy, void* dx, float* dscale, int64_t rows,
                                 int32_t d, int32_t dtype, void* stream) {
  FWD16(spa3d_op_layernorm_bwd, x, scale, stats, dy, dx, dscale, rows, d, dtype, stream)
  if (!x || !scale || !stats || !dy || !dx || !dscale || d <= 0 || d > 2048) return SPA3D_ERR_ARG;
  OpCtx c(stream, nullptr, 0);
  OP_BY_DTYPE(dtype, k_layernorm_bwd<T>(&c, (const T*)x, scale, stats, (const T*)dy, (T*)dx, dscale, rows, d, nullptr));
  return c.status();
}

SPA3D_OP(spa3d_op_attention)(const void* q, const void* k, const void* v, int64_t ldq, int64_t ldk, int64_t ldv, const float* scale_q,
                             const float* scale_k, const float* keymask, int64_t nseq, int32_t Sq, int32_t Sk, int32_t H, int32_t Dh, void* o,
                             float* lse, int32_t dtype, int32_t impl, void* ws, int64_t ws_bytes, void* stream) {
  FWD16(spa3d_op_attention, q, k, v, ldq, ldk, ldv, scale_q, scale_k, keymask, nseq, Sq, Sk, H, Dh, o, lse, dtype, impl, ws, ws_bytes, stream)
  if (!q || !k || !v || !o || !scale_q || !scale_k || Dh > 128) return SPA3D_ERR_ARG;
  OpCtx c(stream, ws, ws_bytes);
  c.attn = AttnPolicy::from_impl(impl);
  const AttnDesc a = op_attn_desc(q, k, v, ldq, ldk, ldv, scale_q, scale_k, keymask, nseq, Sq, Sk, H, Dh, o, lse, dtype);
  OP_BY_DTYPE(dtype, attention_fwd<T>(&c, a));
  return c.status();
}
SPA3D_OP(spa3d_op_attention_holdout)(const void* q, const void* k, const void* v, int64_t ldq, int64_t ldk, int64_t ldv, const float* scale_q,
                                     const float* scale_k, int64_t nseq, int32_t Sq, int32_t Nk, int32_t H, int32_t Dh, const int32_t* holes, void* o,
                                     float* lse, int32_t dtype, int32_t impl, void* ws, int64_t ws_bytes, void* stream) {
  FWD16(spa3d_op_attention_holdout, q, k, v, ldq, ldk, ldv, scale_q, scale_k, nseq, Sq, Nk, H, Dh, holes, o, lse, dtype, impl, ws, ws_bytes, stream)
  if (!q || !k || !v || !o || !scale_q || !scale_k || !holes || Dh < 1 || Dh > 128 || nseq < 1 || nseq > (1 << 20) || Sq < 1 || Nk < 1 || H < 1) return SPA3D_ERR_ARG;
  for (int64_t i = 0; i < nseq; ++i) {
    const int64_t lo = holes[2 * i], hi = holes[2 * i + 1];
    if (lo < 0 || hi > Nk || lo > hi || hi - lo >= Nk) return SPA3D_ERR_ARG;
  }
  OpCtx c(stream, ws, ws_bytes);
  c.attn = AttnPolicy::from_impl(impl);
  int32_t* hd = c.alloc<int32_t>(2 * nseq);
  if (c.ar.overflow) return SPA3D_ERR_WORKSPACE;
  k_set_i32(&c, hd, holes, 2 * nseq);
  AttnDesc a = op_attn_desc(q, k, v, ldq, ldk, ldv, scale_q, scale_k, nullptr, nseq, Sq, 0, H, Dh, o, lse, dtype);
  a.layout = AttnLayout::Hole; a.holes_host = holes; a.holes_dev = hd; a.Nk = Nk;
  OP_BY_DTYPE(dtype, attention_fwd<T>(&c, a));
  return c.status();
}
SPA3D_OP(spa3d_op_attention_bwd)(const void* q, const void* k, const void* v, int64_t ldq, int64_t ldk, int64_t ldv, const float* scale_q,
                                 const float* scale_k, const float* keymask, int64_t nseq, int32_t Sq, int32_t Sk, int32_t H, int32_t Dh,
                                 const void* o, const float* lse, const void* d_o, void* dq, void* dk, void* dv, float* dscale_q,
                                 float* dscale_k, int32_t dtype, int32_t impl, void* ws, int64_t ws_bytes, void* stream) {
  FWD16(spa3d_op_attention_bwd, q, k, v, ldq, ldk, ldv, scale_q, scale_k, keymask, nseq, Sq, Sk, H, Dh, o, lse, d_o, dq, dk, dv, dscale_q, dscale_k, dtype,
        impl, ws, ws_bytes, stream)
  if (!q || !k || !v || !d_o || !dq || !dk || !dv || !dscale_q || !dscale_k || Dh > 128) return SPA3D_ERR_ARG;
  OpCtx c(stream, ws, ws_bytes);
  c.attn = AttnPolicy::from_impl(impl);
  AttnDesc a = op_attn_desc(q, k, v, ldq, ldk, ldv, scale_q, scale_k, keymask, nseq, Sq, Sk, H, Dh, o, lse, dtype);
  op_attn_grads(a, d_o, dq, dk, dv, dscale_q, dscale_k);
  OP_BY_DTYPE(dtype, attention_bwd<T>(&c, a));
  return c.status();
}

static bool ragged_args_ok(const void* const* ptrs, int np, const int32_t* seq_off, int64_t nseq, int64_t ldq, int64_t ldk, int64_t ldv, int32_t S, int32_t H,
                           int32_t Dh, int32_t dtype, int32_t impl) {
  if (!seq_off || dtype != OP_DT16 || Dh != ATTN_DH || S < 2 || S > ATTN_MAX_S || H < 1 || nseq < 1 || nseq > (1 << 20) || nseq * H > 0x7fffffffLL) return false;
  if (impl != 0 && impl != 2 && impl != 3 && impl != 4) return false;
  const int64_t E = (int64_t)H * Dh;
  if (ldq < E || ldk < E || ldv < E || ldq % 8 || ldk % 8 || ldv % 8) return false;
  for (int i = 0; i < np; ++i)
    if (!ptrs[i] || !op_al16(ptrs[i])) return false;
  if (seq_off[0] < 0) return false;
  for (int64_t i = 0; i < nseq; ++i) {
    const int64_t n = (int64_t)seq_off[i + 1] - seq_off[i];
    if (n < 1 || n > S) return false;
  }
  return true;
}
static bool varlen_args_ok(const int32_t* koff, int64_t nseq, int64_t ldq, int64_t ldk, int64_t ldv, int32_t Sq, int32_t H, int32_t Dh, int32_t dtype, int32_t impl) {
  if (!koff || !OP_DTYPE_OK(dtype) || nseq < 1 || nseq > (1 << 20) || Sq < 1 || H < 1 || Dh < 1 || Dh > 128 || impl < 0 || impl > 2) return false;
  if (ldq < (int64_t)H * Dh || ldk < (int64_t)H * Dh || ldv < (int64_t)H * Dh) return false;
  if (impl == 2 && (Dh != ATTN_DH || Sq > ATTN_XCHUNK || dtype == SPA3D_F32 || ldq % 8 || ldk % 8 || ldv % 8)) return false;
  if (koff[0] != 0) return false;
  for (int64_t i = 0; i < nseq; ++i)
    if ((int64_t)koff[i + 1] - koff[i] < 1) return false;
  return true;
}
SPA3D_OP(spa3d_op_attention_ragged)(const void* q, const void* k, const void* v, int64_t ldq, int64_t ldk, int64_t ldv, const float* scale_q,
                                    const float* scale_k, const float* keymask, const int32_t* seq_off, int64_t nseq, int32_t S, int32_t H, int32_t Dh,
                                    void* o, float* lse, int32_t dtype, int32_t impl, void* ws, int64_t ws_bytes, void* stream) {
  FWD16(spa3d_op_attention_ragged, q, k, v, ldq, ldk, ldv, scale_q, scale_k, keymask, seq_off, nseq, S, H, Dh, o, lse, dtype, impl, ws, ws_bytes, stream)
  const void* ptrs[] = {q, k, v, o, scale_q, scale_k};
  if (!ragged_args_ok(ptrs, 6, seq_off, nseq, ldq, ldk, ldv, S, H, Dh, dtype, impl)) return SPA3D_ERR_ARG;
  OpCtx c(stream, ws, ws_bytes);
  c.attn = AttnPolicy::from_impl(impl);
  AttnDesc a = op_attn_desc(q, k, v, ldq, ldk, ldv, scale_q, scale_k, keymask, nseq, S, S, H, Dh, o, lse, dtype);
  a.layout = AttnLayout::RaggedRows; a.total_rows = seq_off[nseq];
  return op_with_offsets(c, seq_off, nseq, &a.seq_off, [&] { attention_fwd<bf16_t>(&c, a); });
}
SPA3D_OP(spa3d_op_attention_ragged_bwd)(const void* q, const void* k, const void* v, int64_t ldq, int64_t ldk, int64_t ldv, const float* scale_q,
// ... 284 lines not shown
```

### include/spa3d.h

```cpp
#ifndef SPA3D_H_
#define SPA3D_H_

#include <stdint.h>

#ifdef __cplusplus
extern "C" {
#endif

#define SPA3D_OK 0
#define SPA3D_ERR_ARG 1
#define SPA3D_ERR_WORKSPACE 2
#define SPA3D_ERR_HIP 3

#define SPA3D_F32 0
#define SPA3D_BF16 1
#define SPA3D_F16 2

typedef struct spa3d_ctx* spa3d_handle;

typedef struct {
  int32_t num_output_frames;
  int32_t num_latent_tokens;
  int32_t latent_token_dim;
  int32_t num_frequencies;
// ... 102 lines not shown
  int32_t resize_h, resize_w;
  const float* scores;
  const float* visible;
  int32_t normalize, use_visibility, colour_bgr, trail, point_size;
  int32_t* pixels;
} spa3d_render;
int64_t spa3d_render_workspace_bytes(spa3d_handle h, int32_t N, int32_t T);
int spa3d_render_tracks(spa3d_handle h, const spa3d_render* r, void* ws, int64_t ws_bytes, void* stream);

typedef struct {
  int32_t n_tracks, T, H, W;
  const float* tracks_2d;
  const float* tracks_3d;
  const float* visible;
  const float* depth_map;
  const float* dino_map; int32_t Hp, Wp;
  const void*  dino_pool;
  const void*  depth_pool;
  const double* intrinsics;
  int32_t n_support, n_query;
  const int32_t *support_index, *query_index, *query_frame;
} spa3d_clip;
int spa3d_build_batch(spa3d_handle h, const spa3d_clip* clips , spa3d_batch* out, void* stream);

int spa3d_loss_and_grads(spa3d_handle h, const float* params, const spa3d_batch* b, float denom,
                         float* grads, int32_t accumulate, float* loss3, spa3d_outputs* out,
                         void* ws, int64_t ws_bytes, void* stream);

#define SPA3D_POS_L1 0
#define SPA3D_POS_HUBER 1
typedef struct {
  float l1_weight, bce_weight;
  int32_t position_kind;
  float huber_delta;
  float axis_weight[3];
  float bce_pos_weight;
} spa3d_loss_config;
int spa3d_set_loss(spa3d_handle h, const spa3d_loss_config* cfg );
int spa3d_get_loss(spa3d_handle h, spa3d_loss_config* out);
int spa3d_set_point_weights(spa3d_handle h, int32_t B, int32_t Q, const float* w );

int spa3d_adamw_step(float* params, const float* grads, float* m, float* v, int64_t n, float lr,
                     int64_t step, float clip, float b1, float b2, float eps, float wd,
                     float* scratch, void* stream);

int spa3d_set_option(spa3d_handle h, const char* name, double value);

int spa3d_set_loss_scale_state(spa3d_handle h, const float* state);

int spa3d_set_counts(spa3d_handle h, int32_t B, const int32_t* support_count, const int32_t* query_count);

int spa3d_grad_segments(spa3d_handle h, int64_t* bounds4);
int spa3d_trainable_range(spa3d_handle h, int64_t* lo_n );
int spa3d_set_grad_events(spa3d_handle h, void* ev_readout, void* ev_latents);
int spa3d_grad_events_recorded(spa3d_handle h, int64_t* out4);
int spa3d_detach(spa3d_handle h, void* ev_readout, void* ev_latents, const float* loss_scale_state);

int spa3d_plan_stats(spa3d_handle h, double* out4);

int spa3d_prof_enable(spa3d_handle h, int32_t on);
int spa3d_prof_read(spa3d_handle h, int32_t cls, double* out4);
int spa3d_prof_dump(spa3d_handle h, const char* path);

int spa3d_uniform_noise(float* out, int64_t n, uint32_t key0, uint32_t key1, void* stream);


int spa3d_op_sin_embed(const float* x, int64_t rows, int32_t C, int32_t nf, void* out, int32_t dtype, void* stream);

int spa3d_op_linear(const void* A, const void* B, const float* bias, const void* residual, void* C,
                    int64_t M, int32_t N, int32_t K, int32_t act, int32_t dtype, int32_t impl,
                    void* ws, int64_t ws_bytes, void* stream);
int spa3d_op_linear_bwd(const void* A, const void* B, const void* dC, void* dA, float* dB, float* dbias,
                        int64_t M, int32_t N, int32_t K, int32_t dtype, int32_t impl,
                        void* ws, int64_t ws_bytes, void* stream);

int spa3d_op_mlp_fused(const void* na, const void* a, const void* w_in, const float* b_in, const void* w_out, const float* b_out,
                       void* y, void* h, void* hpre, int64_t M, int32_t d, int32_t mlp, int32_t dtype,
                       void* ws, int64_t ws_bytes, void* stream);

int spa3d_op_layernorm(const void* x, const float* scale, void* y, float* stats, int64_t rows, int32_t d,
                       int32_t dtype, void* stream);
int spa3d_op_layernorm_bwd(const void* x, const float* scale, const float* stats, const void* dy, void* dx,
                           float* dscale , int64_t rows, int32_t d, int32_t dtype, void* stream);

int spa3d_op_qkv_attention(const void* nq, int64_t ldn, const void* wq, const void* wk, const void* wv, const float* scale_q, const float* scale_k,
                           const float* keymask, const int32_t* seq_off, int64_t nseq, int32_t S, int32_t H, void* qkv, void* o, float* lse,
                           int32_t dtype, void* ws, int64_t ws_bytes, void* stream);

int spa3d_op_attention(const void* q, const void* k, const void* v, int64_t ldq, int64_t ldk, int64_t ldv,
                       const float* scale_q, const float* scale_k, const float* keymask,
                       int64_t nseq, int32_t Sq, int32_t Sk, int32_t H, int32_t Dh, void* o,
                       float* lse ,
                       int32_t dtype, int32_t impl, void* ws, int64_t ws_bytes, void* stream);
int spa3d_op_attention_holdout(const void* q, const void* k, const void* v, int64_t ldq, int64_t ldk, int64_t ldv,
                               const float* scale_q, const float* scale_k, int64_t nseq, int32_t Sq, int32_t Nk,
                               int32_t H, int32_t Dh, const int32_t* holes ,
                               void* o, float* lse, int32_t dtype, int32_t impl,
                               void* ws, int64_t ws_bytes, void* stream);
int spa3d_op_attention_bwd(const void* q, const void* k, const void* v, int64_t ldq, int64_t ldk, int64_t ldv,
                           const float* scale_q, const float* scale_k, const float* keymask,
                           int64_t nseq, int32_t Sq, int32_t Sk, int32_t H, int32_t Dh,
                           const void* o, const float* lse ,
                           const void* d_o, void* dq, void* dk, void* dv, float* dscale_q, float* dscale_k,
                           int32_t dtype, int32_t impl, void* ws, int64_t ws_bytes, void* stream);

int spa3d_op_attention_ragged(const void* q, const void* k, const void* v, int64_t ldq, int64_t ldk, int64_t ldv,
                              const float* scale_q, const float* scale_k, const float* keymask,
                              const int32_t* seq_off , int64_t nseq, int32_t S, int32_t H, int32_t Dh, void* o,
                              float* lse , int32_t dtype, int32_t impl, void* ws, int64_t ws_bytes, void* stream);
int spa3d_op_attention_ragged_bwd(const void* q, const void* k, const void* v, int64_t ldq, int64_t ldk, int64_t ldv,
                                  const float* scale_q, const float* scale_k, const float* keymask,
                                  const int32_t* seq_off , int64_t nseq, int32_t S, int32_t H, int32_t Dh,
                                  const void* o, const float* lse, const void* d_o, void* dq, void* dk, void* dv,
                                  float* dscale_q, float* dscale_k, int32_t dtype, int32_t impl, void* ws, int64_t ws_bytes, void* stream);
int spa3d_op_attention_varlen(const void* q, const void* k, const void* v, int64_t ldq, int64_t ldk, int64_t ldv,
                              const float* scale_q, const float* scale_k, const int32_t* koff ,
                              int64_t nseq, int32_t Sq, int32_t H, int32_t Dh, void* o, float* lse, int32_t dtype, int32_t impl,
                              void* ws, int64_t ws_bytes, void* stream);
int spa3d_op_attention_varlen_bwd(const void* q, const void* k, const void* v, int64_t ldq, int64_t ldk, int64_t ldv,
                                  const float* scale_q, const float* scale_k, const int32_t* koff ,
                                  int64_t nseq, int32_t Sq, int32_t H, int32_t Dh, const void* o, const float* lse, const void* d_o,
                                  void* dq, void* dk, void* dv, float* dscale_q, float* dscale_k, int32_t dtype, int32_t impl,
                                  void* ws, int64_t ws_bytes, void* stream);

int spa3d_op_attention_q1(const void* q0, int64_t ldq0, const void* k, const void* v, int64_t ldk, int64_t ldv,
                          const float* scale_q, const float* scale_k, const float* keymask, const int32_t* seq_off,
                          int64_t nseq, int32_t S, int32_t H, int32_t Dh, void* o0, float* p0, int32_t dtype, void* stream);
int spa3d_op_attention_q1_bwd(const void* q0, int64_t ldq0, const void* k, const void* v, int64_t ldk, int64_t ldv,
                              const float* scale_q, const float* scale_k, const float* keymask, const int32_t* seq_off,
                              int64_t nseq, int32_t S, int32_t H, int32_t Dh, const float* p0, const void* d_o0,
                              void* dq0, void* dk, void* dv, float* dscale_q, float* dscale_k, int32_t dtype, void* stream);

int spa3d_op_rank_linear(const void* x, const void* w, const float* bias, void* out, int64_t M, int32_t N, int32_t K, int64_t ldo,
                         int32_t rgroup, int32_t rskip, int32_t dtype, void* stream);
int spa3d_op_rank_linear_bwd(const void* x, const void* dy, int64_t M, int32_t N, int32_t K, int64_t ldy, int32_t rgroup, int32_t rskip,
                             float* gw, float* gb, int32_t dtype, void* stream);


int spa3d_op_colsum(const void* x, int64_t rows, int32_t n, int64_t ld, int32_t rgroup, int32_t rskip, float* out ,
                    int32_t dtype, void* stream);

enum { SPA3D_ROWS_GATHER_STRIDED = 0, SPA3D_ROWS_GATHER_IDX = 1, SPA3D_ROWS_SCATTER_IDX = 2, SPA3D_ROWS_SCATTER_ADD_IDX = 3, SPA3D_ROWS_ADD_STRIDED = 4 };
int spa3d_op_rows(int32_t mode, const void* src, const int32_t* idx, int64_t stride_rows, void* dst, int64_t n, int32_t d, int32_t dtype, void* stream);

int spa3d_op_prune_plan(const float* km, int64_t nseq, int32_t S, int32_t* cnt, int32_t* seq_off, int32_t* row_src, int64_t* kept, void* stream);

int spa3d_op_share_plan(const int32_t* qframe, int64_t B, int32_t Q, int32_t* slot, int32_t* slot_b, int32_t* slot_f, int32_t* slot_q0, int32_t* scratch,
                        int64_t* nslot, void* stream);

enum { SPA3D_SHARE_ASSEMBLE = 0, SPA3D_SHARE_EXPAND = 1, SPA3D_SHARE_REDUCE = 2 };
int spa3d_op_share_rows(int32_t which, const void* a, const void* b, const int32_t* slot, const int32_t* slot_b, const int32_t* slot_f,
                        const int32_t* slot_q0, int64_t nslot, int64_t B, int32_t Q, int32_t L, int32_t Cl, int32_t d, void* out, int32_t dtype, void* stream);

int spa3d_op_assemble_readout(const void* qtok, const void* lat, const int32_t* qframe, int64_t B, int32_t Q, int32_t L, int32_t Cl, int32_t D, void* seq,
                              int32_t dtype, void* stream);
int spa3d_op_assemble_readout_bwd(const void* dseq, const int32_t* qframe, int64_t B, int32_t Q, int32_t L, int32_t Cl, int32_t D, void* dqtok, float* dlat,
                                  int32_t accumulate, int32_t dtype, void* stream);

int spa3d_op_broadcast_rows(const float* src, int32_t rows, int32_t d, void* dst, int64_t B, int32_t dtype, void* stream);
int spa3d_op_bcast_grad(const void* dsrc, int64_t per, int64_t B, int64_t bstride, float* dparam, int32_t dtype, void* stream);

int spa3d_op_vis_mean_pool(const void* tok, const float* vis, int64_t nseq, int32_t T, int32_t d, void* out, int32_t dtype, void* stream);
int spa3d_op_vis_mean_pool_bwd(const void* dout, const float* vis, int64_t nseq, int32_t T, int32_t d, void* dtok, int32_t dtype, void* stream);


int spa3d_op_sin_embed_scaled(const float* x, int64_t rows, int32_t C, int32_t nf, float prescale, void* out, int32_t dtype, void* stream);
// ... 25 lines not shown
```

Before: 91710.

## Fuse bias-gradient column sums into layernorm backward kernels

The layernorm backward kernels can now also accumulate column sums of the dx they write, rounded to the stored precision, into one or two bias-gradient buffers. These are the gradients for the attention output, cross-attention output and previous block's MLP output biases. The matching weight-gradient GEMMs are told the bias is already done, so they skip fused colsum or a separate colsum pass. This removes extra reads of the gradient tensors, but adds register pressure, shared-memory reductions and extra atomic traffic in the layernorm kernels, and it is controlled by an env or attribute switch that is on by default.

```diff
diff --git a/3dspa_code_amd/_lib.py b/3dspa_code_amd/_lib.py
--- a/3dspa_code_amd/_lib.py
+++ b/3dspa_code_amd/_lib.py
@@ -123,6 +123,7 @@
                                      C.c_void_p]),
     'spa3d_op_layernorm_bwd': (C.c_int, [C.c_void_p, C.c_void_p, C.c_void_p, C.c_void_p, C.c_void_p, C.c_void_p,
                                          C.c_int64, C.c_int32, C.c_int32, C.c_void_p]),
+    'spa3d_op_layernorm_bwd_sums': (C.c_int, [C.c_void_p] * 9 + [C.c_int64, C.c_int32, C.c_int32, C.c_void_p]),
     'spa3d_op_qkv_attention': (C.c_int, [C.c_void_p, C.c_int64] + [C.c_void_p] * 7 + [C.c_int64, C.c_int32, C.c_int32] + [C.c_void_p] * 3
                                + [C.c_int32, C.c_void_p, C.c_int64, C.c_void_p]),
     'spa3d_op_attention': (C.c_int, [C.c_void_p] * 3 + [C.c_int64] * 3 + [C.c_void_p] * 3 + [C.c_int64] + [C.c_int32] * 4
diff --git a/3dspa_code_amd/csrc/common.hpp b/3dspa_code_amd/csrc/common.hpp
--- a/3dspa_code_amd/csrc/common.hpp
+++ b/3dspa_code_amd/csrc/common.hpp
@@ -224,6 +224,7 @@
   const float* pt_w = nullptr; int pt_B = 0, pt_Q = 0;
   int poison = 0;
   int freeze = 0;
+  int bias_sums = 1;
   Prof prof;
 };
 
@@ -324,7 +325,7 @@
 
 template <typename T> void k_layernorm(spa3d_ctx*, const T* x, const float* scale, T* y, float* stats, int64_t rows, int d);
 template <typename T> void k_layernorm_bwd(spa3d_ctx*, const T* x, const float* scale, const float* stats, const T* dy, T* dx,
-                                           float* dscale, int64_t rows, int d, const T* add);
+                                           float* dscale, int64_t rows, int d, const T* add, float* osum0 = nullptr, float* osum1 = nullptr);
 template <typename T> void attention_fwd(spa3d_ctx* c, const AttnDesc& d);
 template <typename T> void attention_bwd(spa3d_ctx* c, const AttnDesc& d);
 void attn_launch(spa3d_ctx* c, const AttnDesc& d, const AttnPlan& pl);
diff --git a/3dspa_code_amd/csrc/layernorm.hip b/3dspa_code_amd/csrc/layernorm.hip
--- a/3dspa_code_amd/csrc/layernorm.hip
+++ b/3dspa_code_amd/csrc/layernorm.hip
@@ -24,15 +24,20 @@
   }
 }
 #define LN_MAXJ 32
-template <typename T>
+template <typename T> __device__ __forceinline__ float as_stored(float v) { if constexpr (sizeof(T) == 4) return v; else return bf2f(f2bf(v)); }
+__device__ __forceinline__ void sink_add(const DetCfg& dc, float* os0, float* os1, int i, float v) {
+  grad_add(dc, os0 + i, v);
+  if (os1) grad_add(dc, os1 + i, v);
+}
+template <typename T, bool SINK>
 __global__ __launch_bounds__(256) void ln_bwd_kernel(const T* __restrict__ x, const float* __restrict__ scale,
                                                      const float* __restrict__ stats, const T* __restrict__ dy, const T* add,
-                                                     T* dx, float* __restrict__ dscale, int64_t rows, int d, const DetCfg* det) {
+                                                     T* dx, float* __restrict__ dscale, int64_t rows, int d, const DetCfg* det, float* os0, float* os1) {
   __shared__ float red[4][64 * LN_MAXJ / 4];
   const int lane = threadIdx.x & 63, w = threadIdx.x >> 6;
-  float acc[LN_MAXJ];
-#pragma unroll
-  for (int j = 0; j < LN_MAXJ; ++j) acc[j] = 0.f;
+  float acc[LN_MAXJ], so[SINK ? LN_MAXJ : 1];
+#pragma unroll
+  for (int j = 0; j < LN_MAXJ; ++j) { acc[j] = 0.f; if constexpr (SINK) so[j] = 0.f; }
   int64_t row = (int64_t)blockIdx.x * 4 + w;
   const int64_t stride = (int64_t)gridDim.x * 4;
   for (; row < rows; row += stride) {
@@ -62,6 +67,7 @@
         float v = r * (g - sg - xh * sgx);
         if (add) v += ld(add + row * d + i);
         st(dxr + i, v);
+        if constexpr (SINK) so[j] += as_stored<T>(v);
       }
     }
   }
@@ -81,7 +87,30 @@
         }
       }
     }
-  }
+    if constexpr (SINK) {
+      __syncthreads();
+#pragma unroll
+      for (int j = 0; j < 8; ++j) red[w][j * 64 + lane] = so[j0 + j];
+      __syncthreads();
+      if (w == 0) {
+#pragma unroll
+        for (int j = 0; j < 8; ++j) {
+          int i = lane + 64 * (j0 + j);
+          if (i < d) sink_add(det_read(det), os0, os1, i, red[0][j * 64 + lane] + red[1][j * 64 + lane] + red[2][j * 64 + lane] + red[3][j * 64 + lane]);
+        }
+      }
+    }
+  }
+}
+template <typename T, int NV>
+__device__ __forceinline__ void store_vec_sum(T* p, const float (&f)[NV], float (&s)[NV]) {
+  if constexpr (sizeof(T) == 4) { *(float4*)p = make_float4(f[0], f[1], f[2], f[3]);
+#pragma unroll
+    for (int i = 0; i < 4; ++i) s[i] += f[i]; }
+  else { unsigned u[4];
+#pragma unroll
+    for (int i = 0; i < 4; ++i) { u[i] = f2bf_pack2(f[2 * i], f[2 * i + 1]); s[2 * i] += unpack_lo(u[i]); s[2 * i + 1] += unpack_hi(u[i]); }
+    *(uint4*)p = make_uint4(u[0], u[1], u[2], u[3]); }
 }
 template <typename T, int NV>
 __device__ __forceinline__ void unpack_vec(const uint4& v, float (&f)[NV]) {
@@ -183,19 +212,28 @@
     }
   }
 }
-template <typename T, int LPR, int CH>
+template <typename T, int LPR, int CH, bool SINK>
 __global__ __launch_bounds__(256) void ln_bwd_part_kernel(const T* __restrict__ x, const float* __restrict__ scale, const float* __restrict__ stats,
                                                           const T* __restrict__ dy, const T* add, T* dx, float* __restrict__ dscale, int64_t rows, int d,
-                                                          const DetCfg* det) {
+                                                          const DetCfg* det, float* os0, float* os1) {
   constexpr int NV = VecOf<T>::N, RPB = 256 / LPR, DV = LPR * CH * NV;
   __shared__ float red[4][DV];
+  __shared__ __attribute__((aligned(16))) float lsc[SINK ? DV : 4];
   const int lane = threadIdx.x & 63, w = threadIdx.x >> 6, sub = threadIdx.x & (LPR - 1);
-  float acc[CH][NV], sc[CH][NV];
+  float acc[CH][NV], sc[SINK ? 1 : CH][NV], so[SINK ? CH : 1][NV];
 #pragma unroll
   for (int c = 0; c < CH; ++c)
 #pragma unroll
-    for (int j = 0; j < NV; ++j) { acc[c][j] = 0.f; sc[c][j] = scale[(sub + LPR * c) * NV + j]; }
+    for (int j = 0; j < NV; ++j) {
+      acc[c][j] = 0.f;
+      if constexpr (SINK) so[c][j] = 0.f; else sc[c][j] = scale[(sub + LPR * c) * NV + j];
+    }
+  if constexpr (SINK) {
+    for (int t = threadIdx.x; t < DV; t += 256) lsc[t] = scale[t];
+    __syncthreads();
+  }
   for (int64_t row = (int64_t)blockIdx.x * RPB + threadIdx.x / LPR; row < rows; row += (int64_t)gridDim.x * RPB) {
+    if constexpr (SINK) asm volatile("" ::: "memory");
     uint4 xr[CH], dr[CH], ar[CH];
     const float mu = stats[row * 2], r = stats[row * 2 + 1];
 #pragma unroll
@@ -209,9 +247,13 @@
     for (int c = 0; c < CH; ++c) {
       float xv[NV], dv[NV];
       unpack_vec<T, NV>(xr[c], xv); unpack_vec<T, NV>(dr[c], dv);
+      if constexpr (SINK) {
+#pragma unroll
+        for (int j = 0; j < NV; j += 4) { const float4 v = *(const float4*)&lsc[(sub + LPR * c) * NV + j]; sc[0][j] = v.x; sc[0][j + 1] = v.y; sc[0][j + 2] = v.z; sc[0][j + 3] = v.w; }
+      }
 #pragma unroll
       for (int j = 0; j < NV; ++j) {
-        xh[c][j] = (xv[j] - mu) * r; gg[c][j] = dv[j] * sc[c][j];
+        xh[c][j] = (xv[j] - mu) * r; gg[c][j] = dv[j] * sc[SINK ? 0 : c][j];
         sg += gg[c][j]; sgx += gg[c][j] * xh[c][j]; acc[c][j] += dv[j] * xh[c][j];
       }
     }
@@ -224,7 +266,8 @@
       unpack_vec<T, NV>(ar[c], av);
 #pragma unroll
       for (int j = 0; j < NV; ++j) o[j] = r * (gg[c][j] - sg - xh[c][j] * sgx) + av[j];
-      store_vec<T, NV>(dx + row * d + (sub + LPR * c) * NV, o);
+      if constexpr (SINK) store_vec_sum<T, NV>(dx + row * d + (sub + LPR * c) * NV, o, so[c]);
+      else store_vec<T, NV>(dx + row * d + (sub + LPR * c) * NV, o);
     }
   }
 #pragma unroll
@@ -238,6 +281,20 @@
     }
   __syncthreads();
   for (int t = threadIdx.x; t < DV; t += 256) grad_add(det_read(det), dscale + t, red[0][t] + red[1][t] + red[2][t] + red[3][t]);
+  if constexpr (SINK) {
+    __syncthreads();
+#pragma unroll
+    for (int c = 0; c < CH; ++c)
+#pragma unroll
+      for (int j = 0; j < NV; ++j) {
+        float a = so[c][j];
+#pragma unroll
+        for (int o = LPR; o < 64; o <<= 1) a += __shfl_xor(a, o, 64);
+        if (lane < LPR) red[w][(sub + LPR * c) * NV + j] = a;
+      }
+    __syncthreads();
+    for (int t = threadIdx.x; t < DV; t += 256) sink_add(det_read(det), os0, os1, t, red[0][t] + red[1][t] + red[2][t] + red[3][t]);
+  }
 }
 template <typename T>
 void k_layernorm(spa3d_ctx* c, const T* x, const float* scale, T* y, float* stats, int64_t rows, int d) {
@@ -265,20 +322,20 @@
   SPA_LAUNCH_CHECK(c);
 }
 
-template <typename T, int STEPS, int U>
+template <typename T, int STEPS, int U, bool SINK>
 __global__ __launch_bounds__(256) void ln_bwd_vec_kernel(const T* __restrict__ x, const float* __restrict__ scale,
                                                          const float* __restrict__ stats, const T* __restrict__ dy, const T* add, T* dx,
-                                                         float* __restrict__ dscale, int64_t rows, int d, const DetCfg* det) {
+                                                         float* __restrict__ dscale, int64_t rows, int d, const DetCfg* det, float* os0, float* os1) {
   constexpr int NV = VecOf<T>::N;
   __shared__ float red[4][64 * NV];
   const int lane = threadIdx.x & 63, w = threadIdx.x >> 6;
   const int nch = d / NV;
-  float acc[STEPS][NV], sc[STEPS][NV];
+  float acc[STEPS][NV], sc[STEPS][NV], so[SINK ? STEPS : 1][NV];
 #pragma unroll
   for (int s_ = 0; s_ < STEPS; ++s_) {
     const int c = lane + 64 * s_;
 #pragma unroll
-    for (int j = 0; j < NV; ++j) { acc[s_][j] = 0.f; sc[s_][j] = c < nch ? scale[c * NV + j] : 0.f; }
+    for (int j = 0; j < NV; ++j) { acc[s_][j] = 0.f; sc[s_][j] = c < nch ? scale[c * NV + j] : 0.f; if constexpr (SINK) so[s_][j] = 0.f; }
   }
   const int64_t stride = (int64_t)gridDim.x * 4;
   for (int64_t row0 = (int64_t)blockIdx.x * 4 + w; row0 < rows; row0 += stride * U) {
@@ -323,7 +380,8 @@
             unpack_vec<T, NV>(ar[u][s_], av);
 #pragma unroll
             for (int j = 0; j < NV; ++j) o[j] = r[u] * (gg[s_][j] - sg - xh[s_][j] * sgx) + av[j];
-            store_vec<T, NV>(dx + row * d + c * NV, o);
+            if constexpr (SINK) store_vec_sum<T, NV>(dx + row * d + c * NV, o, so[s_]);
+            else store_vec<T, NV>(dx + row * d + c * NV, o);
           }
         }
       }
@@ -342,38 +400,59 @@
         for (int j = 0; j < NV; ++j)
           grad_add(det_read(det), dscale + c * NV + j, red[0][lane * NV + j] + red[1][lane * NV + j] + red[2][lane * NV + j] + red[3][lane * NV + j]);
     }
+    if constexpr (SINK) {
+      __syncthreads();
+#pragma unroll
+      for (int j = 0; j < NV; ++j) red[w][lane * NV + j] = so[s_][j];
+      __syncthreads();
+      if (w == 0) {
+        const int c = lane + 64 * s_;
+        if (c < nch)
+#pragma unroll
+          for (int j = 0; j < NV; ++j)
+            sink_add(det_read(det), os0, os1, c * NV + j, red[0][lane * NV + j] + red[1][lane * NV + j] + red[2][lane * NV + j] + red[3][lane * NV + j]);
+      }
+    }
   }
 }
 template <typename T>
 void k_layernorm_bwd(spa3d_ctx* c, const T* x, const float* scale, const float* stats, const T* dy, T* dx, float* dscale,
-                     int64_t rows, int d, const T* add) {
+                     int64_t rows, int d, const T* add, float* osum0, float* osum1) {
   if (c->dry || rows == 0) return;
   ProfScope ps(c, PROF_LN_BWD, 16.0 * (double)rows * d, (double)rows * d * (add ? 4.0 : 3.0) * sizeof(T) + rows * 8.0);
   ps.tag(rows, d, add ? 1 : 0, 0);
+  if (!osum0) std::swap(osum0, osum1);
+  const bool sink = osum0 != nullptr;
   constexpr int gcapb = 1024;
   unsigned g = (unsigned)std::min<int64_t>(cdiv(rows, 4), d <= 512 ? gcapb : 2 * gcapb);
   if (rows <= 16384) g = (unsigned)std::min<int64_t>(g, std::max<int64_t>(64, cdiv(rows, 32)));
   constexpr int NV = VecOf<T>::N;
   const bool al = ((((uintptr_t)x) | ((uintptr_t)dy) | ((uintptr_t)dx) | ((uintptr_t)add)) & 15) == 0;
+#define LN_BWD_LAUNCH(grid, ...)                                                                                                        \
+  do {                                                                                                                                  \
+    if (sink) __VA_ARGS__, true><<<(grid), 256, 0, c->stream>>>(x, scale, stats, dy, add, dx, dscale, rows, d, c->det, osum0, osum1);   \
+    else __VA_ARGS__, false><<<(grid), 256, 0, c->stream>>>(x, scale, stats, dy, add, dx, dscale, rows, d, c->det, nullptr, nullptr);   \
+  } while (0)
   if (d % NV == 0 && al && d <= 64 * NV * 4) {
     const int steps = (d / NV + 63) / 64;
     if constexpr (sizeof(T) == 2) {
-      if (d == 384) { ln_bwd_part_kernel<T, 16, 3><<<(unsigned)std::min<int64_t>(cdiv(rows, 16), 2 * gcapb), 256, 0, c->stream>>>(x, scale, stats, dy, add, dx, dscale, rows, d, c->det); SPA_LAUNCH_CHECK(c); return; }
-      if (d == 1280) { ln_bwd_part_kernel<T, 32, 5><<<(unsigned)std::min<int64_t>(cdiv(rows, 8), 2 * gcapb), 256, 0, c->stream>>>(x, scale, stats, dy, add, dx, dscale, rows, d, c->det); SPA_LAUNCH_CHECK(c); return; }
-    }
-    if (steps == 1) ln_bwd_vec_kernel<T, 1, 1><<<g, 256, 0, c->stream>>>(x, scale, stats, dy, add, dx, dscale, rows, d, c->det);
-    else if (steps == 2) ln_bwd_vec_kernel<T, 2, 2><<<g, 256, 0, c->stream>>>(x, scale, stats, dy, add, dx, dscale, rows, d, c->det);
-    else if (steps == 3) ln_bwd_vec_kernel<T, 3, 2><<<g, 256, 0, c->stream>>>(x, scale, stats, dy, add, dx, dscale, rows, d, c->det);
-    else ln_bwd_vec_kernel<T, 4, 1><<<g, 256, 0, c->stream>>>(x, scale, stats, dy, add, dx, dscale, rows, d, c->det);
+      if (d == 384) { LN_BWD_LAUNCH((unsigned)std::min<int64_t>(cdiv(rows, 16), 2 * gcapb), ln_bwd_part_kernel<T, 16, 3); SPA_LAUNCH_CHECK(c); return; }
+      if (d == 1280) { LN_BWD_LAUNCH((unsigned)std::min<int64_t>(cdiv(rows, 8), 2 * gcapb), ln_bwd_part_kernel<T, 32, 5); SPA_LAUNCH_CHECK(c); return; }
+    }
+    if (steps == 1) LN_BWD_LAUNCH(g, ln_bwd_vec_kernel<T, 1, 1);
+    else if (steps == 2) LN_BWD_LAUNCH(g, ln_bwd_vec_kernel<T, 2, 2);
+    else if (steps == 3) LN_BWD_LAUNCH(g, ln_bwd_vec_kernel<T, 3, 2);
+    else LN_BWD_LAUNCH(g, ln_bwd_vec_kernel<T, 4, 1);
   } else {
-    ln_bwd_kernel<T><<<g, 256, 0, c->stream>>>(x, scale, stats, dy, add, dx, dscale, rows, d, c->det);
-  }
+    LN_BWD_LAUNCH(g, ln_bwd_kernel<T);
+  }
+#undef LN_BWD_LAUNCH
   SPA_LAUNCH_CHECK(c);
 }
 
 #define INST_LN(T) \
   template void k_layernorm<T>(spa3d_ctx*, const T*, const float*, T*, float*, int64_t, int);                                        \
-  template void k_layernorm_bwd<T>(spa3d_ctx*, const T*, const float*, const float*, const T*, T*, float*, int64_t, int, const T*);
+  template void k_layernorm_bwd<T>(spa3d_ctx*, const T*, const float*, const float*, const T*, T*, float*, int64_t, int, const T*, float*, float*);
 INST_LN(float)
 INST_LN(bf16_t)
 }
diff --git a/3dspa_code_amd/csrc/model.hip b/3dspa_code_amd/csrc/model.hip
--- a/3dspa_code_amd/csrc/model.hip
+++ b/3dspa_code_amd/csrc/model.hip
@@ -198,7 +198,7 @@
     d.accumulate = accumulate;
     gemm(d);
   }
-  void lin_bwd_w(const Lin<T>& l, const T* X, const T* dY, int64_t M, int64_t ldx = 0, int brow_group = 0, int brow_skip = 0) {
+  void lin_bwd_w(const Lin<T>& l, const T* X, const T* dY, int64_t M, int64_t ldx = 0, int brow_group = 0, int brow_skip = 0, bool bias_done = false) {
     if constexpr (sizeof(T) == 2) {
       if (l.nseg > 1 && !l.gb && l.gw[0]) {
         GemmDesc d{};
@@ -215,10 +215,11 @@
       d.A = X; d.B = dY + (int64_t)s * l.segw; d.C = l.gw[s]; d.M = l.K; d.N = l.segw; d.K = M;
       d.sAm = 1; d.sAk = ldx ? ldx : l.K; d.sBk = l.N; d.sBn = 1; d.sCm = l.segw;
       d.out_f32 = 1; d.accumulate = 1; d.zero_page = zero_page; d.brow_group = brow_group; d.brow_skip = brow_skip;
-      d.colsum_out = l.gb ? l.gb + (int64_t)s * l.segw : nullptr;
+      float* gb = bias_done ? nullptr : l.gb;
+      d.colsum_out = gb ? gb + (int64_t)s * l.segw : nullptr;
       const GemmKernel k = plan(d);
       gemm_launch<T>(c, d, k);
-      if (l.gb && !gemm_tn_fuses_colsum(k, d)) k_colsum<T>(c, dY + (int64_t)s * l.segw, M, l.segw, l.N, l.gb + (int64_t)s * l.segw, brow_group, brow_skip);
+      if (gb && !gemm_tn_fuses_colsum(k, d)) k_colsum<T>(c, dY + (int64_t)s * l.segw, M, l.segw, l.N, l.gb + (int64_t)s * l.segw, brow_group, brow_skip);
     }
   }
 
@@ -300,20 +301,25 @@
               st->st1 = st1; st->st2 = st2; st->cq = cq; st->ckv = ckv; st->co = co; st->lse = lse; st->clse = clse; st->shared = sh != nullptr; }
     else c->ar.release(mk);
   }
+  float* sums_to(const Lin<T>& l) const { return c->bias_sums ? l.gb : nullptr; }
+  float* dx_sums_of(const XfW<T>& x, int i) const { return i > 0 ? sums_to(x.blocks[i - 1].mlp_out) : nullptr; }
+  bool dy_sums_done(const XfW<T>& x, int i, int top) const { return i < top && sums_to(x.blocks[i].mlp_out) != nullptr; }
   void block_bwd(const BlockW<T>& w, const BlockStash<T>& s, const T* dy, T* dx, int64_t nseq, int S, const float* km, const T* kv,
-                 int Skv, T* dkv, const Rag& rg = Rag(), const Share<T>* sh = nullptr, const int32_t* koff_h = nullptr, const int32_t* koff_d = nullptr) {
+                 int Skv, T* dkv, const Rag& rg = Rag(), const Share<T>* sh = nullptr, const int32_t* koff_h = nullptr, const int32_t* koff_d = nullptr,
+                 float* dx_sums = nullptr, bool dy_bias_done = false) {
     const int64_t M = rg.off ? rg.rows : nseq * S, Mg = rg.off ? (M + 7) & ~int64_t(7) : M; const int d = w.d;
     int64_t mk = c->ar.mark();
-    lin_bwd_w(w.mlp_out, s.h, dy, M);
+    lin_bwd_w(w.mlp_out, s.h, dy, M, 0, 0, 0, dy_bias_done);
     T* dh = alloc<T>(Mg * w.mlp);
     lin_bwd_x(w.mlp_out, dy, dh, Mg, s.hpre);
     lin_bwd_w(w.mlp_in, s.na, dh, M);
     T* dna = alloc<T>(Mg * d);
     lin_bwd_x(w.mlp_in, dh, dna, Mg);
     T* da = alloc<T>(Mg * d);
-    k_layernorm_bwd<T>(c, s.a, w.norm_attn, s.st2, dna, da, w.g_norm_attn, M, d, dy);
+    float* const da_sums[2] = {sums_to(w.out), w.cross ? sums_to(w.cout) : nullptr};
+    k_layernorm_bwd<T>(c, s.a, w.norm_attn, s.st2, dna, da, w.g_norm_attn, M, d, dy, da_sums[0], da_sums[1]);
     T* dnq = dna;
-    lin_bwd_w(w.out, s.o, da, M);
+    lin_bwd_w(w.out, s.o, da, M, 0, 0, 0, da_sums[0] != nullptr);
     T* d_o = alloc<T>(Mg * E);
     lin_bwd_x(w.out, da, d_o, Mg);
     T* dqkv = alloc<T>(Mg * 3 * E);
@@ -340,7 +346,7 @@
     lin_bwd_w(w.qkv, s.nq, dqkv, M);
     lin_bwd_x(w.qkv, dqkv, dnq, Mg);
     if (w.cross) {
-      lin_bwd_w(w.cout, s.co, da, M);
+      lin_bwd_w(w.cout, s.co, da, M, 0, 0, 0, da_sums[1] != nullptr);
       lin_bwd_x(w.cout, da, d_o, M);
       T* dcq = dqkv;
       const int64_t nkv = koff_h ? koff_h[nseq] : nseq * Skv;
@@ -351,7 +357,7 @@
       lin_bwd_w(w.ckv, kv, dckv, nkv);
       lin_bwd_x(w.ckv, dckv, dkv, nkv, nullptr, 1);
     }
-    k_layernorm_bwd<T>(c, s.x, w.norm_q, s.st1, dnq, dx, w.g_norm_q, M, d, da);
+    k_layernorm_bwd<T>(c, s.x, w.norm_q, s.st1, dnq, dx, w.g_norm_q, M, d, da, dx_sums);
     c->ar.release(mk);
   }
 
@@ -399,8 +405,9 @@
     T* dna = alloc<T>(nseq * d);
     lin_bwd_x(w.mlp_in, dh, dna, nseq);
     T* da0 = alloc<T>(nseq * d);
-    k_layernorm_bwd<T>(c, s.a0, w.norm_attn, s.st2, dna, da0, w.g_norm_attn, nseq, d, dy0);
-    lin_bwd_w(w.out, s.o0, da0, nseq);
+    float* const da_sums = sums_to(w.out);
+    k_layernorm_bwd<T>(c, s.a0, w.norm_attn, s.st2, dna, da0, w.g_norm_attn, nseq, d, dy0, da_sums);
+    lin_bwd_w(w.out, s.o0, da0, nseq, 0, 0, 0, da_sums != nullptr);
     T* d_o0 = alloc<T>(nseq * E);
     lin_bwd_x(w.out, da0, d_o0, nseq);
     T* dq0 = alloc<T>(nseq * E); T* dkv = alloc<T>(Mg * 2 * E);
@@ -704,7 +711,8 @@
       const int nro = (int)ro.blocks.size();
       block_bwd_last(ro.blocks[nro - 1], k.ro_lst, dq0, dseq, nq, S, nullptr);
       for (int i = nro - 2; i >= 0; --i)
-        block_bwd(ro.blocks[i], k.ro_st[i], dseq, dseq, nq, S, nullptr, nullptr, 0, nullptr, Rag(), (i == 0 && k.ro_share) ? &k.ro_sh : nullptr);
+        block_bwd(ro.blocks[i], k.ro_st[i], dseq, dseq, nq, S, nullptr, nullptr, 0, nullptr, Rag(), (i == 0 && k.ro_share) ? &k.ro_sh : nullptr, nullptr, nullptr,
+                  dx_sums_of(ro, i), dy_sums_done(ro, i, nro - 2));
       if (k.packed) {
         for (int64_t s = 0; s < k.Bc; ++s) {
           const int64_t q0 = k.qoff[s]; const int qs = k.qoff[s + 1] - k.qoff[s];
@@ -728,7 +736,8 @@
       k_layernorm_bwd<T>(c, k.dec_last, dec.norm_enc, k.st_dec, dlatd, ddec, dec.g_norm_enc, nl, Cl, nullptr);
     }
     for (int i = (int)dec.blocks.size() - 1; i >= 0; --i)
-      block_bwd(dec.blocks[i], k.dec_st[i], ddec, ddec, k.Bc, L, nullptr, nullptr, 0, nullptr);
+      block_bwd(dec.blocks[i], k.dec_st[i], ddec, ddec, k.Bc, L, nullptr, nullptr, 0, nullptr, Rag(), nullptr, nullptr, nullptr,
+                dx_sums_of(dec, i), dy_sums_done(dec, i, (int)dec.blocks.size() - 1));
     lin_bwd_w(decomp, k.lat_qT, ddec, nl);
     T* dlq = alloc<T>(nl * Ld);
     lin_bwd_x(decomp, ddec, dlq, nl);
@@ -745,7 +754,8 @@
     T* denc_out = alloc<T>(nkeys * d);
     k_zero(c, denc_out, nkeys * d * (int64_t)sizeof(T));
     for (int i = (int)t2l.blocks.size() - 1; i >= 0; --i)
-      block_bwd(t2l.blocks[i], k.t2l_st[i], dt2l, dt2l, k.Bc, L, nullptr, k.enc_out, k.Nk, denc_out, Rag(), nullptr, k.packed ? k.noff.data() : nullptr, k.koff_dev);
+      block_bwd(t2l.blocks[i], k.t2l_st[i], dt2l, dt2l, k.Bc, L, nullptr, k.enc_out, k.Nk, denc_out, Rag(), nullptr, k.packed ? k.noff.data() : nullptr, k.koff_dev,
+                dx_sums_of(t2l, i), dy_sums_done(t2l, i, (int)t2l.blocks.size() - 1));
     grad_segment_done(1);
     if (lat0_trains) k_bcast_grad<T>(c, dt2l, (int64_t)L * dl, k.Bc, (int64_t)L * dl, g_lat0);
     return denc_out;
@@ -762,7 +772,8 @@
       k_vis_mean_pool_bwd<T>(c, denc_out, k.sup_vis, nseq, T_, d, dln);
       k_layernorm_bwd<T>(c, k.enc_last, enc.norm_enc, k.st_all, dln, dtok, enc.g_norm_enc, nseq * S, d, nullptr);
       for (int i = nenc - 1; i >= 0; --i)
-        block_bwd(enc.blocks[i], k.enc_st[i], dtok, dtok, nseq, S, k.km, nullptr, 0, nullptr);
+        block_bwd(enc.blocks[i], k.enc_st[i], dtok, dtok, nseq, S, k.km, nullptr, 0, nullptr, Rag(), nullptr, nullptr, nullptr,
+                  dx_sums_of(enc, i), dy_sums_done(enc, i, nenc - 1));
       lin_bwd_w(tok, k.sinbuf, dtok, nseq * T_);
     } else {
       T* dr0 = alloc<T>(nseq * d);
@@ -771,7 +782,8 @@
       const float* km = rg.off ? nullptr : k.km;
       block_bwd_last(enc.blocks[nenc - 1], k.enc_lst, dr0, dtok, nseq, S, km, rg);
       for (int i = nenc - 2; i >= 0; --i)
-        block_bwd(enc.blocks[i], k.enc_st[i], dtok, dtok, nseq, S, km, nullptr, 0, nullptr, rg);
+        block_bwd(enc.blocks[i], k.enc_st[i], dtok, dtok, nseq, S, km, nullptr, 0, nullptr, rg, nullptr, nullptr, nullptr,
+                  dx_sums_of(enc, i), dy_sums_done(enc, i, nenc - 2));
       const T* dtok_dense = dtok;
       if (rg.off) {
         T* d0 = alloc<T>(nseq * d);
@@ -1219,6 +1231,7 @@
   e = getenv("SPA3D_QUERY_CHUNK"); if (e) c->query_chunk = std::max(0, atoi(e));
   e = getenv("SPA3D_TRACK_CHUNK"); if (e) c->track_chunk = std::max(0, atoi(e));
   e = getenv("SPA3D_FREEZE"); if (e && atoi(e) >= 0 && atoi(e) <= 2) c->freeze = atoi(e);
+  e = getenv("SPA3D_BIAS_SUMS"); if (e) c->bias_sums = atoi(e) != 0;
   *out = c;
   return SPA3D_OK;
 }
@@ -1373,6 +1386,7 @@
   const std::string n(name);
   if (n == "prune") h->prune = value != 0;
   else if (n == "ro_share") h->ro_share = value != 0;
+  else if (n == "bias_sums") h->bias_sums = value != 0;
   else if (n == "loss_scale") { if (h->cfg.precision != SPA3D_F16) { h->err = "loss_scale applies to SPA3D_F16 handles only"; return SPA3D_ERR_ARG; } h->loss_scale = (float)value; }
   else if (n == "attn_impl") h->attn = AttnPolicy::from_impl((int)value);
   else if (n == "gemm_impl") set_gemm_impl(h, (int)value);
diff --git a/3dspa_code_amd/csrc/ops.hip b/3dspa_code_amd/csrc/ops.hip
--- a/3dspa_code_amd/csrc/ops.hip
+++ b/3dspa_code_amd/csrc/ops.hip
@@ -202,6 +202,14 @@
   OP_BY_DTYPE(dtype, k_layernorm_bwd<T>(&c, (const T*)x, scale, stats, (const T*)dy, (T*)dx, dscale, rows, d, nullptr));
   return c.status();
 }
+SPA3D_OP(spa3d_op_layernorm_bwd_sums)(const void* x, const float* scale, const float* stats, const void* dy, const void* add, void* dx, float* dscale,
+                                      float* osum0, float* osum1, int64_t rows, int32_t d, int32_t dtype, void* stream) {
+  FWD16(spa3d_op_layernorm_bwd_sums, x, scale, stats, dy, add, dx, dscale, osum0, osum1, rows, d, dtype, stream)
+  if (!x || !scale || !stats || !dy || !dx || !dscale || !OP_DTYPE_OK(dtype) || rows < 0 || d <= 0 || d > 2048) return SPA3D_ERR_ARG;
+  OpCtx c(stream, nullptr, 0);
+  OP_BY_DTYPE(dtype, k_layernorm_bwd<T>(&c, (const T*)x, scale, stats, (const T*)dy, (T*)dx, dscale, rows, d, (const T*)add, osum0, osum1));
+  return c.status();
+}
 
 SPA3D_OP(spa3d_op_attention)(const void* q, const void* k, const void* v, int64_t ldq, int64_t ldk, int64_t ldv, const float* scale_q,
                              const float* scale_k, const float* keymask, int64_t nseq, int32_t Sq, int32_t Sk, int32_t H, int32_t Dh, void* o,
diff --git a/include/spa3d.h b/include/spa3d.h
--- a/include/spa3d.h
+++ b/include/spa3d.h
@@ -208,6 +208,9 @@
                        int32_t dtype, void* stream);
 int spa3d_op_layernorm_bwd(const void* x, const float* scale, const float* stats, const void* dy, void* dx,
                            float* dscale , int64_t rows, int32_t d, int32_t dtype, void* stream);
+int spa3d_op_layernorm_bwd_sums(const void* x, const float* scale, const float* stats, const void* dy, const void* add, void* dx,
+                                float* dscale , float* osum0, float* osum1, int64_t rows, int32_t d, int32_t dtype,
+                                void* stream);
 
 int spa3d_op_qkv_attention(const void* nq, int64_t ldn, const void* wq, const void* wk, const void* wv, const float* scale_q, const float* scale_k,
                            const float* keymask, const int32_t* seq_off, int64_t nseq, int32_t S, int32_t H, void* qkv, void* o, float* lse,
```

New measurement: 92110, median of 6. No clear change (+0.4%).
